# nubot-nudt/RDMNet

Hardware: AMD Instinct MI355X
Metric: scan-pairs/sec (whole node) (higher is better)
Workload: dtype f32

## Files before the change

include/rdmnet_hip.h:

```cpp
#ifndef RDMNET_HIP_H_
#define RDMNET_HIP_H_

#include <stddef.h>
#include <stdint.h>

#ifdef __cplusplus
extern "C" {
#endif

#define RDM_ABI_VERSION 2

int rdm_abi_version(void);
size_t rdm_abi_struct_size(int which);
const char* rdm_last_error(void);

int rdm_rehash_schedule(int64_t max_elems, int64_t* at_host, int64_t* buckets_host, int cap);

size_t rdm_grid_subsample_workspace_bytes(int64_t n_points, int batch);
int rdm_grid_subsample(const float* points, int64_t n_points, const int64_t* lengths, int batch,
                       float voxel_size, float* out_points, int64_t* out_lengths, void* ws,
                       size_t ws_bytes, void* stream);
int rdm_grid_subsample_form(const float* points, int64_t n_points, const int64_t* lengths, int batch, float voxel_size,
                            float* out_points, int64_t* out_lengths, void* ws, size_t ws_bytes, void* stream, int form);

// ... 51 lines not shown
size_t rdm_information_workspace_bytes(int64_t n_q, int64_t n_s);
int rdm_information_matrix(const float* q, int64_t n_q, int64_t ld_q, const float* s, int64_t n_s, int64_t ld_s,
                           const double* q_transform_host, const double* s_transform_host, double cell, double radius,
                           double* out_host, int64_t* corr_out, int64_t capacity, void* ws, size_t ws_bytes, void* stream);

size_t rdm_pose_graph_workspace_bytes(int64_t n_graphs, int64_t n_nodes, int64_t n_edges);
size_t rdm_pose_graph_workspace_bytes_pc(int64_t n_graphs, int64_t n_nodes, int64_t n_edges, int preconditioner);
int rdm_pose_graph_optimize_pc(int64_t n_graphs, const int64_t* graph_node_offsets_host, const int64_t* graph_edge_offsets_host,
                               const double* nodes, const int64_t* edges_host, const double* transforms, const double* informations,
                               const uint8_t* uncertain_host, double line_process_weight, double edge_prune_threshold,
                               int max_iterations, double gradient_tolerance, double cost_tolerance, int pcg_max_iterations,
                               double pcg_tolerance, int preconditioner, double* nodes_out, double* weights_out,
                               uint8_t* pruned_out, double* report_host, void* ws, size_t ws_bytes, void* stream);
int rdm_pose_graph_optimize(int64_t n_graphs, const int64_t* graph_node_offsets_host, const int64_t* graph_edge_offsets_host,
                            const double* nodes, const int64_t* edges_host, const double* transforms, const double* informations,
                            const uint8_t* uncertain_host, double line_process_weight, double edge_prune_threshold,
                            int max_iterations, double gradient_tolerance, double cost_tolerance, int pcg_max_iterations,
                            double pcg_tolerance, double* nodes_out, double* weights_out, uint8_t* pruned_out, double* report_host,
                            void* ws, size_t ws_bytes, void* stream);
int rdm_pose_graph_edge_terms_host(const double* source_pose, const double* target_pose, const double* transform,
                                   const double* information, double line_process_weight, int uncertain, double* out);
int rdm_pose_graph_retract_host(const double* pose, const double* delta, double* out);
int rdm_pose_graph_chain_host(int64_t n, const double* diag, const double* off, const double* rhs, double* out);
size_t rdm_pose_graph_workspace_bytes_ls(int64_t n_graphs, const int64_t* graph_node_offsets_host,
                                         const int64_t* graph_edge_offsets_host, const int64_t* edges_host, int preconditioner,
                                         int linear_solver);
int rdm_pose_graph_optimize_ls(int64_t n_graphs, const int64_t* graph_node_offsets_host, const int64_t* graph_edge_offsets_host,
                               const double* nodes, const int64_t* edges_host, const double* transforms, const double* informations,
                               const uint8_t* uncertain_host, double line_process_weight, double edge_prune_threshold,
                               int max_iterations, double gradient_tolerance, double cost_tolerance, int pcg_max_iterations,
                               double pcg_tolerance, int preconditioner, int linear_solver, double* nodes_out, double* weights_out,
                               uint8_t* pruned_out, double* report_host, void* ws, size_t ws_bytes, void* stream);
int rdm_pose_graph_direct_max_separator(void);
int64_t rdm_pose_graph_separator_host(int64_t n_nodes, int64_t n_edges, const int64_t* edges_host, int64_t* out_nodes,
                                      int64_t capacity);
int rdm_pose_graph_direct_host(int64_t n_nodes, int64_t n_edges, const int64_t* edges_host, const double* diag, const double* off,
                               const double* rhs, double* out);

size_t rdm_gemm_workspace_bytes(int64_t m, int64_t n, int batches);
int rdm_gemm(const float* a, int64_t lda, int64_t stride_a, const float* b, int64_t ldb,
             int64_t stride_b, int trans_b, float* c, int64_t ldc, int64_t stride_c, int64_t m,
             int64_t n, int64_t k, int batches, const float* bias, const float* rowdiv, int act,
             void* ws, size_t ws_bytes, void* stream);
int rdm_gemm_last_plan(int* out4_host);

int rdm_kpconv_gather(const float* q_points, int64_t m, const float* s_points, int64_t n_s,
                      const float* s_feats, int64_t c, int64_t ldf, const uint8_t* s_positive,
                      const int64_t* idx, int64_t h, int64_t ldi, const int32_t* width,
                      const float* kernel_points, float sigma, float* wf, int64_t ldw, float* nn,
                      void* stream);
int rdm_kpconv_fused_enabled(void);
int rdm_kpconv_fused_supported(int64_t c_in, int64_t c_out);
int64_t rdm_kpconv_fused_partial_rows(int64_t m, int64_t c_in);
size_t rdm_kpconv_packed_floats(int64_t c_in, int64_t c_out);
int rdm_kpconv_pack_weights(const float* w_host, int64_t c_in, int64_t c_out, float* packed_host);
int rdm_kpconv_fused(const float* q_points, int64_t m, const float* s_points, int64_t n_s, const float* s_feats,
                     int64_t c, int64_t ldf, const uint8_t* s_positive, const int64_t* idx, int64_t h, int64_t ldi,
                     const int32_t* width, const float* kernel_points, float sigma, const float* w_packed,
                     const float* bias, int64_t c_out, float* out, int64_t ldo, double* gn_partial,
                     const float* order_records, void* stream);
int rdm_kpconv_fused_form(const float* q_points, int64_t m, const float* s_points, int64_t n_s, const float* s_feats,
                          int64_t c, int64_t ldf, const uint8_t* s_positive, const int64_t* idx, int64_t h, int64_t ldi,
                          const int32_t* width, const float* kernel_points, float sigma, const float* w_packed,
                          const float* bias, int64_t c_out, float* out, int64_t ldo, double* gn_partial,
                          const float* order_records, int form, void* stream);
size_t rdm_kpconv_fused_workspace_bytes(int64_t m, int64_t c_in, int64_t c_out);
int rdm_kpconv_fused_group_norm(const float* q_points, int64_t m, const float* s_points, int64_t n_s,
                                const float* s_feats, int64_t c, int64_t ldf, const uint8_t* s_positive,
                                const int64_t* idx, int64_t h, int64_t ldi, const int32_t* width,
                                const float* kernel_points, float sigma, const float* w_packed, const float* bias,
                                int64_t c_out, int groups, const float* gamma, const float* beta, float eps, int act,
                                float* conv_out, int64_t ld_conv, float* y, int64_t ldy, void* ws, size_t ws_bytes,
                                const float* order_records, void* stream);
int rdm_kpconv_gather_ordered(const float* q_points, int64_t m, const float* s_points, int64_t n_s,
                              const float* s_feats, int64_t c, int64_t ldf, const uint8_t* s_positive,
                              const int64_t* idx, int64_t h, int64_t ldi, const int32_t* width,
                              const float* kernel_points, float sigma, float* wf, int64_t ldw, float* nn,
                              const float* order_records, void* stream);
int rdm_kpconv_gather_form(const float* q_points, int64_t m, const float* s_points, int64_t n_s,
                              const float* s_feats, int64_t c, int64_t ldf, const uint8_t* s_positive,
                              const int64_t* idx, int64_t h, int64_t ldi, const int32_t* width,
                              const float* kernel_points, float sigma, float* wf, int64_t ldw, float* nn,
                              const float* order_records, int form, void* stream);
int rdm_row_positive(const float* x, int64_t n, int64_t c, int64_t ld, uint8_t* out, void* stream);

size_t rdm_group_norm_workspace_bytes(int64_t n, int64_t c);
int rdm_group_norm(const float* x, int64_t n, int64_t c, int64_t ldx, int groups, const float* gamma,
                   const float* beta, float eps, const float* residual, int64_t ldr, int act, float* y,
                   int64_t ldy, uint8_t* positive, void* ws, size_t ws_bytes, void* stream);
int rdm_group_norm_form(const float* x, int64_t n, int64_t c, int64_t ldx, int groups, const float* gamma,
                        const float* beta, float eps, const float* residual, int64_t ldr, int act, float* y, int64_t ldy,
                        uint8_t* positive, void* ws, size_t ws_bytes, int form, void* stream);
size_t rdm_linear_group_norm_workspace_bytes(int64_t m, int64_t n);
int rdm_linear_group_norm(const float* x, int64_t ldx, const float* w, int64_t ldw, const float* bias,
                          const float* rowdiv, int64_t m, int64_t n, int64_t k, int groups, const float* gamma,
                          const float* beta, float eps, const float* residual, int64_t ldr, int act, float* lin_out,
                          int64_t ld_lin, float* y, int64_t ldy, uint8_t* positive, void* ws, size_t ws_bytes,
                          void* stream);
int rdm_patch_scores(const float* ref_feats, int64_t ld_ref, int64_t n_ref, const int64_t* ref_idx, const float* src_feats,
                     int64_t ld_src, int64_t n_src, const int64_t* src_idx, int64_t batch, int64_t side, int64_t d,
                     const float* rowdiv, float* scores, void* stream);
size_t rdm_decoder_stage_workspace_bytes(int64_t m, int64_t n, int64_t k);
int rdm_decoder_stage(const float* coarse, int64_t n_coarse, int64_t c1, int64_t ld1, const int64_t* idx, int64_t ldi,
                      const float* skip, int64_t c2, int64_t ld2, int64_t m, const float* w, int64_t ldw, const float* bias,
                      int64_t n, int groups, const float* gamma, const float* beta, float eps, int act, float* lin_out,
                      int64_t ld_lin, float* y, int64_t ldy, void* ws, size_t ws_bytes, void* stream);
int rdm_layer_norm(const float* x, int64_t n, int64_t c, int64_t ldx, const float* residual,
                   int64_t ldr, const float* gamma, const float* beta, float eps, int act, float* y,
                   int64_t ldy, void* stream);
int rdm_linear_layer_norm(const float* x, int64_t ldx, const float* w, int64_t ldw, const float* bias, int64_t m, int64_t n,
                          int64_t k, const float* residual, int64_t ldr, const float* gamma, const float* beta, float eps,
                          int act, float* y, int64_t ldy, void* stream);
int rdm_attention_tail(const float* hidden, int64_t ld_hidden, const float* x, int64_t ldx, int64_t m, int64_t d,
                       const float* wo, int64_t ld_wo, const float* bo, const float* gamma1, const float* beta1,
                       const float* w1, int64_t ld_w1, const float* b1, const float* w2, int64_t ld_w2, const float* b2,
                       const float* gamma2, const float* beta2, float eps, float* out, int64_t ld_out, void* stream);
size_t rdm_attention_tail_packed_floats(void);
int rdm_attention_tail_pack_weights(const float* wo, int64_t ld_wo, const float* w1, int64_t ld_w1, const float* w2, int64_t ld_w2,
                                    float* packed, void* stream);
int rdm_attention_tail_packed(const float* hidden, int64_t ld_hidden, const float* x, int64_t ldx, int64_t m, int64_t d,
                              const float* packed, const float* bo, const float* gamma1, const float* beta1, const float* b1,
                              const float* b2, const float* gamma2, const float* beta2, float eps, float* out, int64_t ld_out,
                              void* stream);
int rdm_gather_max(const float* x, int64_t n_s, int64_t c, int64_t ldx, const int64_t* idx, int64_t m,
                   int64_t h, int64_t ldi, const int32_t* width, float* y, int64_t ldy, void* stream);
int rdm_gather_rows(const void* x, int64_t n_src, int64_t words, int64_t ldx, const int64_t* idx, int64_t m,
                    void* y, int64_t ldy, void* stream);
int rdm_upsample_concat(const float* coarse, int64_t n_coarse, int64_t c1, int64_t ld1,
                        const int64_t* idx, int64_t ldi, const float* skip, int64_t c2, int64_t ld2,
                        int64_t m, float* y, int64_t ldy, void* stream);

int rdm_rope(float* q, int64_t ldq, float* k, int64_t ldk, const float* emb, int64_t lde, int64_t n,
             int64_t d_model, void* stream);
int rdm_attention(const float* q, int64_t ldq, const float* k, int64_t ldk, const float* v, int64_t ldv,
                  float* out, int64_t ldo, int64_t n_q, int64_t n_k, int heads, int head_dim, void* stream);
int rdm_attention_bf16(const float* q, int64_t ldq, const float* k, int64_t ldk, const float* v, int64_t ldv,
                  float* out, int64_t ldo, int64_t n_q, int64_t n_k, int heads, int head_dim, void* stream);
int rdm_attention_self_pair(const float* q, int64_t ldq, const float* k, int64_t ldk, const float* v, int64_t ldv,
                            float* out, int64_t ldo, int64_t n0, int64_t n1, int heads, int head_dim, int bf16,
                            void* stream);
int rdm_attention_topk(const float* q, int64_t ldq, const float* k, int64_t ldk, const float* v, int64_t ldv, float* out,
                       int64_t ldo, int64_t n_q, int64_t n_k, int64_t keep, int heads, int head_dim, void* stream);
int rdm_attention_self_pair_topk(const float* q, int64_t ldq, const float* k, int64_t ldk, const float* v, int64_t ldv,
                                 float* out, int64_t ldo, int64_t n0, int64_t n1, int64_t keep0, int64_t keep1, int heads,
                                 int head_dim, void* stream);
int64_t rdm_topk_count(int64_t n, double frac);

int rdm_vote_shift(const float* xyz, const float* offsets, int64_t ldo, int64_t n, float lx, float ly,
                   float lz, float* out, void* stream);
int rdm_sigmoid_column(const float* x, int64_t ldx, int64_t n, float* out, void* stream);
int rdm_l2_normalize(const float* x, int64_t ldx, int64_t n, int64_t c, float* y, int64_t ldy, void* stream);

int rdm_nms(const int64_t* idx, int64_t n, int64_t h, int64_t ldi, const int32_t* width, uint8_t* keep,
            void* stream);
int rdm_compact_indices(const uint8_t* keep, int64_t begin, int64_t end, int32_t* order, int32_t* count,
                        void* stream);

size_t rdm_point_to_node_workspace_bytes(int64_t n_points, int64_t n_nodes);
int rdm_point_to_node(const float* points, int64_t n_points, const float* nodes, int64_t n_nodes, int k,
                      int64_t* knn_idx, uint8_t* knn_mask, uint8_t* node_mask, int32_t* status, void* ws,
                      size_t ws_bytes, void* stream);
int rdm_point_to_node_pair(const float* points_a, int64_t n_a, const float* nodes_a, int64_t m_a, const float* points_b,
                           int64_t n_b, const float* nodes_b, int64_t m_b, int k, int64_t* knn_idx_a, uint8_t* knn_mask_a,
                           uint8_t* node_mask_a, int64_t* knn_idx_b, uint8_t* knn_mask_b, uint8_t* node_mask_b,
                           int32_t* status, void* ws, size_t ws_bytes, void* stream);

// ... 76 lines not shown
  int sinkhorn_iterations;
  float acceptance_radius;
  int correspondence_threshold;
  int num_refinement_steps;
  int use_vote;
  int attention_bf16;
  size_t arena_bytes;
} rdm_engine_config;

typedef struct rdm_engine_result {
  float transform[16];
  int32_t n_correspondences, n_hypotheses, best_hypothesis;
  int64_t n_ref_nodes, n_src_nodes, n_node_correspondences;
  int64_t level_sizes[5];
  int64_t level_ref_sizes[5];
  const float* ref_corr_points;
  const float* src_corr_points;
  const float* corr_scores;
  const float* transform_dev;
  size_t arena_used;
  const float* host_ref_corr_points;
  const float* host_src_corr_points;
  const float* host_corr_scores;
  int32_t n_host_correspondences;
} rdm_engine_result;

typedef struct rdm_tensor_view {
  void* data;
  int64_t rows, cols, ld;
  int dtype;
} rdm_tensor_view;

typedef struct rdm_kpconv_profile {
  int64_t m, h, c_in, c_out, pooled_channels;
  float gather_ms;
  float total_ms;
  int32_t fused;
  int32_t reserved;
} rdm_kpconv_profile;

int rdm_engine_create(const rdm_engine_config* cfg, rdm_engine** out);
void rdm_engine_destroy(rdm_engine* e);
int rdm_engine_set_param(rdm_engine* e, const char* name, const float* data_host, const int64_t* shape_host, int ndim);
int rdm_engine_finalize(rdm_engine* e);
int rdm_engine_share_params(rdm_engine* e, const rdm_engine* src);
int rdm_engine_run(rdm_engine* e, const float* ref_points, int64_t n_ref, const float* src_points, int64_t n_src,
                   rdm_engine_result* result_host, void* stream);

typedef struct rdm_data_dict {
  const float* features;  int64_t features_ld;
  const float* points[5];
  const int64_t* lengths[5];
  int64_t n_points[5], n_ref[5];
  const int64_t* neighbors[5];   int64_t neighbors_width[5],   neighbors_ld[5];   const int32_t* neighbors_count[5];
  const int64_t* subsampling[4]; int64_t subsampling_width[4], subsampling_ld[4]; const int32_t* subsampling_count[4];
  const int64_t* upsampling[4];  int64_t upsampling_width[4],  upsampling_ld[4];  const int32_t* upsampling_count[4];
  const int32_t* collate_status; int64_t n_collate_status;
} rdm_data_dict;

int rdm_engine_collate(rdm_engine* e, const float* ref_points, int64_t n_ref, const float* src_points, int64_t n_src,
                       rdm_engine_result* result_host, void* stream);

int rdm_engine_forward(rdm_engine* e, const rdm_data_dict* data, rdm_engine_result* result_host, void* stream);

int rdm_engine_collate_batch(rdm_engine* e, int n_pairs, const float* const* ref_points, const int64_t* n_ref,
                             const float* const* src_points, const int64_t* n_src, void* stream);
int rdm_engine_forward_batched(rdm_engine* e, int k, rdm_engine_result* result_host, void* stream);

int rdm_engine_run_lockstep(rdm_engine* const* engines, int n_pairs, const float* const* ref_points, const int64_t* n_ref,
                            const float* const* src_points, const int64_t* n_src, rdm_engine_result* const* results,
                            int collate_batched, void* stream);
int rdm_engine_forward_lockstep(rdm_engine* const* engines, int n_pairs, const rdm_data_dict* const* data,
                                rdm_engine_result* const* results, void* stream);
int rdm_engine_collate_lockstep(rdm_engine* const* engines, int n_pairs, const float* const* ref_points, const int64_t* n_ref,
                                const float* const* src_points, const int64_t* n_src, rdm_engine_result* const* results, void* stream);
void rdm_lockstep_stats(long long* out, int reset);
int rdm_lockstep_selftest(int n_ctx, const int* script, int len, int* log, int cap, int* rcs);
int rdm_lockstep_selftest_gpu(int n_ctx, const int* script, int len, int threads, int32_t* out, int64_t cap_slots, void* stream);
void rdm_lockstep_stats_dump(void);
int rdm_engine_reserve(rdm_engine* e, size_t bytes);
int rdm_engine_set_wait(rdm_engine* e, int sleep_us);
int rdm_engine_set_pairs_in_flight(rdm_engine* e, int n);
int rdm_engine_set_overlap(rdm_engine* e, int mode);
int rdm_engine_set_attention_topk(rdm_engine* e, int n_layers, const double* fracs);
int rdm_engine_set_fine_matching(rdm_engine* e, const rdm_fine_matching_options* options);
int rdm_engine_enable_profile(rdm_engine* e, int enable);
int rdm_engine_get_profile(rdm_engine* e, rdm_kpconv_profile* out, int cap);
int rdm_engine_keep_taps(rdm_engine* e, int enable);
int rdm_engine_get_tensor(rdm_engine* e, const char* name, rdm_tensor_view* out);
int rdm_engine_export(rdm_engine* e, int n, const char* const* names, void* const* dst, void* stream);
int rdm_engine_describe(rdm_engine* e, int n, const char* const* names, rdm_tensor_view* out);
int rdm_engine_gt_node_correspondences(rdm_engine* e, const float* transform, double pos_radius, int64_t* out_indices,
                                       float* out_overlaps, int64_t capacity, int64_t* count_host, void* stream);
int rdm_engine_feature_correspondences(rdm_engine* e, int level, int mode, int64_t* ref_idx, int64_t* src_idx, float* ref_points,
                                       float* src_points, float* dists, int64_t capacity, int64_t* count_host, void* stream);
int rdm_engine_gt_point_correspondences_count(rdm_engine* e, int level, const double* transform_host, double radius,
                                              int64_t* totals_host, void* stream);
int rdm_engine_gt_point_correspondences_fill(rdm_engine* e, int64_t* out, int64_t capacity, void* stream);
int rdm_engine_alignment_quality(rdm_engine* e, int level, const double* transform_host, double radius, double* out_host,
                                 void* stream);
int rdm_engine_information_matrix(rdm_engine* e, int level, const double* transform_host, double radius, double* out_host,
                                  int64_t* corr_out, int64_t capacity, void* stream);
int rdm_copy_device(void* dst, const void* src, size_t bytes, void* stream);

#define RDM_EVAL_RECORD_WIDTH 20
enum { RDM_EVAL_LGR = 0, RDM_EVAL_SVD = 1, RDM_EVAL_RANSAC = 2 };
typedef struct rdm_eval_options {
  int32_t method;
  int32_t num_corr;
  double acceptance_radius;
  float ransac_distance_threshold;
  int32_t ransac_n;
  int32_t ransac_iterations;
  int32_t reserved;
  uint64_t ransac_seed;
} rdm_eval_options;
size_t rdm_eval_pairs_workspace_bytes(int64_t num_pairs, int64_t total_corr, int64_t max_corr, const rdm_eval_options* options);
int rdm_eval_pairs(int64_t num_pairs, const int64_t* corr_offsets, const int64_t* corr_offsets_host, const float* ref_corr,
                   const float* src_corr, const float* corr_scores, const float* gt_transform, float* est_transform,
                   const int64_t* node_offsets, const int64_t* ref_node_corr, const int64_t* src_node_corr,
                   const int64_t* gt_offsets, const int64_t* gt_node_corr, const int64_t* node_dims,
                   const rdm_eval_options* options, double* records, void* ws, size_t ws_bytes, void* stream);

#define RDM_ROBUST_MAX_CORR 16384
#define RDM_ROBUST_STATS 6
enum { RDM_ROBUST_CLIQUE = 0, RDM_ROBUST_KCORE = 1, RDM_ROBUST_NONE = 2 };
int64_t rdm_robust_default_clique_nodes(void);
size_t rdm_robust_registration_workspace_bytes(int64_t n_corr, int inlier_selection);
int rdm_robust_registration(const float* src_corr, const float* ref_corr, int64_t n_corr, double noise_bound, double cbar2,
                            double gnc_factor, int max_iterations, double cost_threshold, int inlier_selection,
                            int64_t max_clique_nodes, double* transform, int32_t* stats, int32_t* selected, double* weights,
                            int64_t weights_capacity, int32_t* degree, int32_t* core, void* ws, size_t ws_bytes, void* stream);

#define RDM_SCAN_CONTEXT_MAX_DIM 64
#define RDM_SCAN_CONTEXT_LD 64
size_t rdm_scan_context_workspace_bytes(int64_t n_scans, int n_rings, int n_sectors);
int rdm_scan_context(const float* points, int64_t ld, int64_t n_points, const int64_t* offsets, int64_t n_scans, int n_rings,
                     int n_sectors, double max_range, double lidar_height, float* desc, float* desc_norm, uint64_t* valid, void* ws,
                     size_t ws_bytes, void* stream);
size_t rdm_scan_context_distance_workspace_bytes(int64_t n_q, int64_t n_c, int n_rings, int n_sectors);
int rdm_scan_context_distance(const float* q_desc, int64_t n_q, const float* c_desc, int64_t n_c, int n_rings, int n_sectors,
                              int64_t q_base, int64_t c_base, int64_t exclude_recent, float* best_distance, int32_t* best_index,
                              int32_t* best_shift, float* dist, int32_t* shift, void* ws, size_t ws_bytes, void* stream);

#define RDM_VOXEL_MAP_FRAC_BITS 20
#define RDM_VOXEL_MAP_MAX_CHANNELS 8
#define RDM_VOXEL_MAP_STATS 6
size_t rdm_voxel_map_bytes(int64_t capacity, int channels);
int rdm_voxel_map_reset(void* map, size_t map_bytes, int64_t capacity, int channels, void* stream);
int rdm_voxel_map_integrate(void* map, size_t map_bytes, int64_t capacity, int channels, double voxel, const float* points, int64_t ld,
                            int64_t total, const int64_t* offsets, const double* poses, int64_t n_scans, double min_range,
                            double max_range, void* stream);
int rdm_voxel_map_rehash(const void* old_map, size_t old_bytes, int64_t old_capacity, void* new_map, size_t new_bytes,
                         int64_t new_capacity, int channels, void* stream);
int rdm_voxel_map_stats(const void* map, size_t map_bytes, int64_t capacity, int channels, uint64_t* stats, void* stream);
size_t rdm_voxel_map_extract_workspace_bytes(int64_t capacity);
int rdm_voxel_map_extract(const void* map, size_t map_bytes, int64_t capacity, int channels, double voxel, int64_t min_points,
                          float* points, int32_t* counts, int32_t* cells, int64_t max_rows, int64_t* n_rows, void* ws, size_t ws_bytes,
                          void* stream);

#define RDM_VOXEL_MOMENTS_PLANES 9
#define RDM_VOXEL_MOMENTS_SHIFT 8
size_t rdm_voxel_moments_bytes(int64_t capacity);
int rdm_voxel_moments_reset(void* moments, size_t moments_bytes, int64_t capacity, void* stream);
int rdm_voxel_map_integrate_moments(void* map, size_t map_bytes, int64_t capacity, int channels, double voxel, const float* points,
                                    int64_t ld, int64_t total, const int64_t* offsets, const double* poses, int64_t n_scans,
// ... 38 lines not shown
```

rdmnet_amd/_lib.py:

```python
import ctypes
import os

_HERE = os.path.dirname(os.path.abspath(__file__))
LIB_PATH = os.environ.get('RDM_LIB_PATH') or os.path.join(_HERE, 'librdmnet_hip.so')

c_void = ctypes.c_void_p
c_i64 = ctypes.c_int64
c_int = ctypes.c_int
c_f32 = ctypes.c_float
c_size = ctypes.c_size_t

ABI_VERSION = 2


class FineMatchingOptions(ctypes.Structure):
    _fields_ = [('topk', ctypes.c_int32), ('mutual', ctypes.c_int32), ('use_dustbin', ctypes.c_int32),
                ('use_global_score', ctypes.c_int32), ('confidence_threshold', ctypes.c_float),
                ('correspondence_limit', ctypes.c_int32)]

    @classmethod
    def of(cls, topk=1, mutual=False, use_dustbin=True, confidence_threshold=0.0, use_global_score=False,
           correspondence_limit=None):
        return cls(int(topk), int(bool(mutual)), int(bool(use_dustbin)), int(bool(use_global_score)), float(confidence_threshold),
                   0 if correspondence_limit is None else int(correspondence_limit))


class EvalOptions(ctypes.Structure):
    METHODS = {'lgr': 0, 'svd': 1, 'ransac': 2}
    _fields_ = [('method', ctypes.c_int32), ('num_corr', ctypes.c_int32), ('acceptance_radius', ctypes.c_double),
                ('ransac_distance_threshold', ctypes.c_float), ('ransac_n', ctypes.c_int32),
                ('ransac_iterations', ctypes.c_int32), ('reserved', ctypes.c_int32), ('ransac_seed', ctypes.c_uint64)]

    @classmethod
    def of(cls, method='lgr', num_corr=None, acceptance_radius=0.6, distance_threshold=0.3, ransac_n=4, num_iterations=50000,
           seed=0):
        if method not in cls.METHODS:
            raise ValueError(f'Unsupported registration method: {method}.')
        return cls(cls.METHODS[method], 0 if num_corr is None else int(num_corr), float(acceptance_radius),
                   float(distance_threshold), int(ransac_n), int(num_iterations), 0, int(seed))


ROBUST_SELECTIONS = {'clique': 0, 'kcore': 1, 'none': 2}
ROBUST_MAX_CORR = 16384
ROBUST_STATS = ('num_selected', 'valid', 'exact', 'iterations', 'translation_inliers', 'edges')

SCAN_CONTEXT_MAX_DIM = 64
SCAN_CONTEXT_LD = 64

VOXEL_MAP_FRAC_BITS = 20
VOXEL_MAP_MAX_CHANNELS = 8
VOXEL_MAP_STATS = ('occupied', 'integrated', 'skipped_nonfinite', 'skipped_range', 'out_of_extent', 'dropped_full')
VOXEL_MOMENTS_PLANES = 9
VOXEL_OBSERVATIONS_MAX_SCANS = 64

EVAL_RECORD_WIDTH = 20
EVAL_FIELDS = ('num_corr', 'residual', 'inlier_ratio', 'inlier_ratio_0.3', 'inlier_ratio_0.1', 'overlap', 'precision', 'rre', 'rte',
               'rx', 'ry', 'rz', 'inliers', 'inliers_0.3', 'inliers_0.1', 'overlap_rows', 'hit_cells', 'pred_cells', 'gt_cells',
               'bad_indices')

SIGNATURES = {
    'rdm_abi_version': (c_int, []),
    'rdm_abi_struct_size': (c_size, [c_int]),
    'rdm_last_error': (ctypes.c_char_p, []),
    'rdm_rehash_schedule': (c_int, [c_i64, c_void, c_void, c_int]),
    'rdm_grid_subsample_workspace_bytes': (c_size, [c_i64, c_int]),
    'rdm_grid_subsample': (c_int, [c_void, c_i64, c_void, c_int, c_f32, c_void, c_void, c_void, c_size,
                                   c_void]),
    'rdm_grid_subsample_form': (c_int, [c_void, c_i64, c_void, c_int, c_f32, c_void, c_void, c_void, c_size,
                                        c_void, c_int]),
    'rdm_radius_neighbors_workspace_bytes': (c_size, [c_i64, c_i64, c_int]),
    'rdm_radius_neighbors': (c_int, [c_void, c_i64, c_void, c_i64, c_void, c_void, c_int, c_f32, c_int,
                                     c_void, c_void, c_void, c_void, c_void, c_size, c_void]),
    'rdm_radius_grid_workspace_bytes': (c_size, [c_i64]),
    'rdm_radius_grid_build': (c_int, [c_void, c_i64, c_void, c_int, c_f32, c_void, c_size, c_void]),
    'rdm_radius_grid_query': (c_int, [c_void, c_size, c_i64, c_void, c_i64, c_void, c_int, c_f32, c_int, c_void, c_void,
                                      c_void, c_void, c_void, c_size, c_void]),
    'rdm_gemm_workspace_bytes': (c_size, [c_i64, c_i64, c_int]),
    'rdm_gemm': (c_int, [c_void, c_i64, c_i64, c_void, c_i64, c_i64, c_int, c_void, c_i64, c_i64, c_i64, c_i64,
                         c_i64, c_int, c_void, c_void, c_int, c_void, c_size, c_void]),
    'rdm_gemm_last_plan': (c_int, [c_void]),
    'rdm_kpconv_gather': (c_int, [c_void, c_i64, c_void, c_i64, c_void, c_i64, c_i64, c_void, c_void, c_i64,
                                  c_i64, c_void, c_void, c_f32, c_void, c_i64, c_void, c_void]),
    'rdm_kpconv_gather_ordered': (c_int, [c_void, c_i64, c_void, c_i64, c_void, c_i64, c_i64, c_void, c_void, c_i64,
                                          c_i64, c_void, c_void, c_f32, c_void, c_i64, c_void, c_void, c_void]),
    'rdm_kpconv_gather_form': (c_int, [c_void, c_i64, c_void, c_i64, c_void, c_i64, c_i64, c_void, c_void, c_i64,
                                       c_i64, c_void, c_void, c_f32, c_void, c_i64, c_void, c_void, c_int, c_void]),
    'rdm_kpconv_fused_enabled': (c_int, []),
    'rdm_kpconv_fused_supported': (c_int, [c_i64, c_i64]),
    'rdm_kpconv_fused_partial_rows': (c_i64, [c_i64, c_i64]),
    'rdm_kpconv_packed_floats': (c_size, [c_i64, c_i64]),
    'rdm_kpconv_pack_weights': (c_int, [c_void, c_i64, c_i64, c_void]),
    'rdm_kpconv_fused': (c_int, [c_void, c_i64, c_void, c_i64, c_void, c_i64, c_i64, c_void, c_void, c_i64, c_i64, c_void, c_void,
                                 c_f32, c_void, c_void, c_i64, c_void, c_i64, c_void, c_void, c_void]),
    'rdm_kpconv_fused_form': (c_int, [c_void, c_i64, c_void, c_i64, c_void, c_i64, c_i64, c_void, c_void, c_i64, c_i64, c_void, c_void,
                                      c_f32, c_void, c_void, c_i64, c_void, c_i64, c_void, c_void, c_int, c_void]),
    'rdm_kpconv_fused_workspace_bytes': (c_size, [c_i64, c_i64, c_i64]),
    'rdm_kpconv_fused_group_norm': (c_int, [c_void, c_i64, c_void, c_i64, c_void, c_i64, c_i64, c_void, c_void, c_i64, c_i64, c_void,
                                            c_void, c_f32, c_void, c_void, c_i64, c_int, c_void, c_void, c_f32, c_int, c_void, c_i64,
                                            c_void, c_i64, c_void, c_size, c_void, c_void]),
    'rdm_voxel_downsample_workspace_bytes': (c_size, [c_i64]),
    'rdm_voxel_downsample': (c_int, [c_void, c_i64, c_i64, c_int, ctypes.c_double, c_void, c_i64, c_void, c_void, c_void,
                                     c_size, c_void]),
    'rdm_ransac_workspace_bytes': (c_size, [c_int]),
    'rdm_ransac_correspondences': (c_int, [c_void, c_void, c_i64, c_f32, c_int, c_int, ctypes.c_uint64, c_void, c_void, c_void,
                                           c_void, c_void, c_size, c_void]),
    'rdm_icp_workspace_bytes': (c_size, [c_i64, c_i64]),
    'rdm_icp_point_to_point': (c_int, [c_void, c_i64, c_i64, c_void, c_i64, c_i64, ctypes.c_double, c_void, c_int, ctypes.c_double,
                                       ctypes.c_double, c_void, c_void, c_void, c_void, c_void, c_size, c_void]),
    'rdm_icp_correspondences': (c_int, [c_void, c_i64, c_void, c_i64, c_i64, ctypes.c_double, c_void, c_void, c_void, c_size,
                                        c_void]),
    'rdm_ball_workspace_bytes': (c_size, [c_i64, c_i64]),
    'rdm_ball_count': (c_int, [c_void, c_i64, c_i64, c_void, c_i64, c_i64, c_void, ctypes.c_double, c_void, c_void, c_void, c_void,
                               c_void, c_size, c_void]),
    'rdm_ball_fill': (c_int, [c_void, c_i64, c_i64, c_i64, c_void, c_i64, c_void, c_size, c_void]),
    'rdm_nearest_workspace_bytes': (c_size, [c_i64, c_i64]),
    'rdm_nearest': (c_int, [c_void, c_i64, c_i64, c_void, c_i64, c_i64, c_void, c_void, ctypes.c_double, ctypes.c_double, c_void,
                            c_void, c_void, c_void, c_size, c_void]),
    'rdm_realign_error': (c_int, [c_void, c_i64, c_i64, c_void, c_void, c_void, c_void, c_size, c_void]),
    'rdm_information_workspace_bytes': (c_size, [c_i64, c_i64]),
    'rdm_information_matrix': (c_int, [c_void, c_i64, c_i64, c_void, c_i64, c_i64, c_void, c_void, ctypes.c_double, ctypes.c_double,
                                       c_void, c_void, c_i64, c_void, c_size, c_void]),
    'rdm_pose_graph_workspace_bytes': (c_size, [c_i64, c_i64, c_i64]),
    'rdm_pose_graph_optimize': (c_int, [c_i64, c_void, c_void, c_void, c_void, c_void, c_void, c_void, ctypes.c_double, ctypes.c_double,
                                        c_int, ctypes.c_double, ctypes.c_double, c_int, ctypes.c_double, c_void, c_void, c_void, c_void,
                                        c_void, c_size, c_void]),
    'rdm_pose_graph_workspace_bytes_pc': (c_size, [c_i64, c_i64, c_i64, c_int]),
    'rdm_pose_graph_optimize_pc': (c_int, [c_i64, c_void, c_void, c_void, c_void, c_void, c_void, c_void, ctypes.c_double,
                                           ctypes.c_double, c_int, ctypes.c_double, ctypes.c_double, c_int, ctypes.c_double, c_int,
                                           c_void, c_void, c_void, c_void, c_void, c_size, c_void]),
    'rdm_pose_graph_chain_host': (c_int, [c_i64, c_void, c_void, c_void, c_void]),
    'rdm_pose_graph_workspace_bytes_ls': (c_size, [c_i64, c_void, c_void, c_void, c_int, c_int]),
    'rdm_pose_graph_optimize_ls': (c_int, [c_i64, c_void, c_void, c_void, c_void, c_void, c_void, c_void, ctypes.c_double,
                                           ctypes.c_double, c_int, ctypes.c_double, ctypes.c_double, c_int, ctypes.c_double, c_int, c_int,
                                           c_void, c_void, c_void, c_void, c_void, c_size, c_void]),
    'rdm_pose_graph_direct_max_separator': (c_int, []),
    'rdm_pose_graph_separator_host': (c_i64, [c_i64, c_i64, c_void, c_void, c_i64]),
    'rdm_pose_graph_direct_host': (c_int, [c_i64, c_i64, c_void, c_void, c_void, c_void, c_void]),
    'rdm_pose_graph_edge_terms_host': (c_int, [c_void, c_void, c_void, c_void, ctypes.c_double, c_int, c_void]),
    'rdm_pose_graph_retract_host': (c_int, [c_void, c_void, c_void]),
    'rdm_neighbor_histogram': (c_int, [c_void, c_i64, c_void, c_int, c_void]),
    'rdm_radius_grid_records': (c_void, [c_void, c_size, c_i64]),
    'rdm_row_positive': (c_int, [c_void, c_i64, c_i64, c_i64, c_void, c_void]),
    'rdm_group_norm_workspace_bytes': (c_size, [c_i64, c_i64]),
    'rdm_group_norm': (c_int, [c_void, c_i64, c_i64, c_i64, c_int, c_void, c_void, c_f32, c_void, c_i64, c_int,
                               c_void, c_i64, c_void, c_void, c_size, c_void]),
    'rdm_group_norm_form': (c_int, [c_void, c_i64, c_i64, c_i64, c_int, c_void, c_void, c_f32, c_void, c_i64, c_int,
                                    c_void, c_i64, c_void, c_void, c_size, c_int, c_void]),
    'rdm_linear_group_norm_workspace_bytes': (c_size, [c_i64, c_i64]),
    'rdm_linear_group_norm': (c_int, [c_void, c_i64, c_void, c_i64, c_void, c_void, c_i64, c_i64, c_i64, c_int, c_void, c_void,
                                      c_f32, c_void, c_i64, c_int, c_void, c_i64, c_void, c_i64, c_void, c_void, c_size, c_void]),
    'rdm_patch_scores': (c_int, [c_void, c_i64, c_i64, c_void, c_void, c_i64, c_i64, c_void, c_i64, c_i64, c_i64, c_void, c_void,
                                 c_void]),
    'rdm_decoder_stage_workspace_bytes': (c_size, [c_i64, c_i64, c_i64]),
    'rdm_decoder_stage': (c_int, [c_void, c_i64, c_i64, c_i64, c_void, c_i64, c_void, c_i64, c_i64, c_i64, c_void, c_i64, c_void,
                                  c_i64, c_int, c_void, c_void, c_f32, c_int, c_void, c_i64, c_void, c_i64, c_void, c_size, c_void]),
    'rdm_layer_norm': (c_int, [c_void, c_i64, c_i64, c_i64, c_void, c_i64, c_void, c_void, c_f32, c_int, c_void,
                               c_i64, c_void]),
    'rdm_linear_layer_norm': (c_int, [c_void, c_i64, c_void, c_i64, c_void, c_i64, c_i64, c_i64, c_void, c_i64, c_void, c_void,
                                      c_f32, c_int, c_void, c_i64, c_void]),
    'rdm_attention_tail': (c_int, [c_void, c_i64, c_void, c_i64, c_i64, c_i64, c_void, c_i64, c_void, c_void, c_void, c_void, c_i64,
                                   c_void, c_void, c_i64, c_void, c_void, c_void, c_f32, c_void, c_i64, c_void]),
    'rdm_attention_tail_packed_floats': (c_size, []),
    'rdm_attention_tail_pack_weights': (c_int, [c_void, c_i64, c_void, c_i64, c_void, c_i64, c_void, c_void]),
    'rdm_attention_tail_packed': (c_int, [c_void, c_i64, c_void, c_i64, c_i64, c_i64, c_void, c_void, c_void, c_void, c_void, c_void,
                                          c_void, c_void, c_f32, c_void, c_i64, c_void]),
    'rdm_gather_max': (c_int, [c_void, c_i64, c_i64, c_i64, c_void, c_i64, c_i64, c_i64, c_void, c_void, c_i64,
                               c_void]),
    'rdm_upsample_concat': (c_int, [c_void, c_i64, c_i64, c_i64, c_void, c_i64, c_void, c_i64, c_i64, c_i64,
                                    c_void, c_i64, c_void]),
    'rdm_gather_rows': (c_int, [c_void, c_i64, c_i64, c_i64, c_void, c_i64, c_void, c_i64, c_void]),
    'rdm_rope': (c_int, [c_void, c_i64, c_void, c_i64, c_void, c_i64, c_i64, c_i64, c_void]),
    'rdm_attention': (c_int, [c_void, c_i64, c_void, c_i64, c_void, c_i64, c_void, c_i64, c_i64, c_i64, c_int, c_int,
                              c_void]),
    'rdm_attention_bf16': (c_int, [c_void, c_i64, c_void, c_i64, c_void, c_i64, c_void, c_i64, c_i64, c_i64, c_int, c_int,
                              c_void]),
    'rdm_attention_self_pair': (c_int, [c_void, c_i64, c_void, c_i64, c_void, c_i64, c_void, c_i64, c_i64, c_i64, c_int, c_int,
                                        c_int, c_void]),
    'rdm_attention_topk': (c_int, [c_void, c_i64, c_void, c_i64, c_void, c_i64, c_void, c_i64, c_i64, c_i64, c_i64, c_int, c_int,
                                   c_void]),
    'rdm_attention_self_pair_topk': (c_int, [c_void, c_i64, c_void, c_i64, c_void, c_i64, c_void, c_i64, c_i64, c_i64, c_i64, c_i64,
                                             c_int, c_int, c_void]),
    'rdm_topk_count': (c_i64, [c_i64, ctypes.c_double]),
    'rdm_vote_shift': (c_int, [c_void, c_void, c_i64, c_i64, c_f32, c_f32, c_f32, c_void, c_void]),
    'rdm_sigmoid_column': (c_int, [c_void, c_i64, c_i64, c_void, c_void]),
    'rdm_l2_normalize': (c_int, [c_void, c_i64, c_i64, c_i64, c_void, c_i64, c_void]),
    'rdm_nms': (c_int, [c_void, c_i64, c_i64, c_i64, c_void, c_void, c_void]),
    'rdm_compact_indices': (c_int, [c_void, c_i64, c_i64, c_void, c_void, c_void]),
    'rdm_point_to_node_workspace_bytes': (c_size, [c_i64, c_i64]),
    'rdm_point_to_node': (c_int, [c_void, c_i64, c_void, c_i64, c_int, c_void, c_void, c_void, c_void, c_void,
                                  c_size, c_void]),
    'rdm_point_to_node_pair': (c_int, [c_void, c_i64, c_void, c_i64, c_void, c_i64, c_void, c_i64, c_int, c_void, c_void, c_void,
                                       c_void, c_void, c_void, c_void, c_void, c_size, c_void]),
    'rdm_coarse_matching_workspace_bytes': (c_size, [c_i64, c_i64]),
    'rdm_coarse_matching': (c_int, [c_void, c_i64, c_i64, c_i64, c_void, c_void, c_int, c_int, c_void, c_void, c_void,
                                    c_void, c_void, c_size, c_void]),
    'rdm_coarse_matching_features_workspace_bytes': (c_size, [c_i64, c_i64]),
    'rdm_coarse_matching_features': (c_int, [c_void, c_i64, c_i64, c_void, c_i64, c_i64, c_i64, c_void, c_void, c_int, c_int,
                                             c_void, c_void, c_void, c_void, c_void, c_size, c_void]),
    'rdm_gt_node_correspondences_workspace_bytes': (c_size, [c_i64, c_i64]),
    'rdm_gt_node_correspondences': (c_int, [c_void, c_i64, c_void, c_i64, c_void, c_void, c_i64, c_void, c_void, c_i64, c_int,
                                            c_void, c_void, c_void, c_void, c_void, ctypes.c_double, c_void, c_void, c_i64,
                                            c_void, c_void, c_void, c_size, c_void]),
    'rdm_sinkhorn': (c_int, [c_void, c_i64, c_i64, c_i64, c_void, c_void, c_void, c_int, c_void, c_void]),
    'rdm_lgr_workspace_bytes': (c_size, [c_i64]),
    'rdm_lgr': (c_int, [c_void, c_void, c_void, c_void, c_void, c_i64, c_i64, c_f32, c_int, c_int, c_void, c_void,
                        c_void, c_void, c_void, c_void, c_size, c_void]),
    'rdm_lgr_options_capacity': (c_i64, [c_i64, c_i64, c_void]),
    'rdm_lgr_options_workspace_bytes': (c_size, [c_i64, c_i64, c_void]),
    'rdm_lgr_options': (c_int, [c_void, c_i64, c_void, c_void, c_void, c_void, c_void, c_i64, c_i64, c_f32, c_int, c_int, c_void,
                                c_void, c_void, c_void, c_void, c_void, c_void, c_size, c_void]),
    'rdm_engine_create': (c_int, [c_void, c_void]),
    'rdm_engine_destroy': (None, [c_void]),
    'rdm_engine_set_param': (c_int, [c_void, ctypes.c_char_p, c_void, c_void, c_int]),
    'rdm_engine_finalize': (c_int, [c_void]),
    'rdm_engine_share_params': (c_int, [c_void, c_void]),
    'rdm_engine_run': (c_int, [c_void, c_void, c_i64, c_void, c_i64, c_void, c_void]),
    'rdm_engine_collate': (c_int, [c_void, c_void, c_i64, c_void, c_i64, c_void, c_void]),
    'rdm_engine_forward': (c_int, [c_void, c_void, c_void, c_void]),
    'rdm_engine_collate_batch': (c_int, [c_void, c_int, c_void, c_void, c_void, c_void, c_void]),
    'rdm_engine_forward_batched': (c_int, [c_void, c_int, c_void, c_void]),
    'rdm_engine_run_lockstep': (c_int, [c_void, c_int, c_void, c_void, c_void, c_void, c_void, c_int, c_void]),
    'rdm_engine_forward_lockstep': (c_int, [c_void, c_int, c_void, c_void, c_void]),
    'rdm_engine_collate_lockstep': (c_int, [c_void, c_int, c_void, c_void, c_void, c_void, c_void, c_void]),
    'rdm_lockstep_stats': (None, [c_void, c_int]),
    'rdm_lockstep_stats_dump': (None, []),
    'rdm_lockstep_selftest': (c_int, [c_int, c_void, c_int, c_void, c_int, c_void]),
    'rdm_lockstep_selftest_gpu': (c_int, [c_int, c_void, c_int, c_int, c_void, c_i64, c_void]),
    'rdm_engine_reserve': (c_int, [c_void, c_size]),
    'rdm_engine_set_wait': (c_int, [c_void, c_int]),
    'rdm_engine_set_pairs_in_flight': (c_int, [c_void, c_int]),
    'rdm_engine_set_overlap': (c_int, [c_void, c_int]),
    'rdm_engine_set_attention_topk': (c_int, [c_void, c_int, c_void]),
    'rdm_engine_set_fine_matching': (c_int, [c_void, c_void]),
    'rdm_engine_enable_profile': (c_int, [c_void, c_int]),
    'rdm_engine_get_profile': (c_int, [c_void, c_void, c_int]),
    'rdm_engine_keep_taps': (c_int, [c_void, c_int]),
    'rdm_engine_get_tensor': (c_int, [c_void, ctypes.c_char_p, c_void]),
    'rdm_engine_describe': (c_int, [c_void, c_int, c_void, c_void]),
    'rdm_engine_export': (c_int, [c_void, c_int, c_void, c_void, c_void]),
    'rdm_engine_gt_node_correspondences': (c_int, [c_void, c_void, ctypes.c_double, c_void, c_void, c_i64, c_void, c_void]),
    'rdm_feature_match_workspace_bytes': (c_size, [c_i64, c_i64, c_int]),
    'rdm_feature_match': (c_int, [c_void, c_i64, c_i64, c_void, c_i64, c_i64, c_i64, c_int, c_void, c_void, c_void, c_void, c_void,
                                  c_void, c_size, c_void]),
    'rdm_feature_match_select': (c_int, [c_int, c_void, c_void, c_void, c_void, c_i64, c_i64, c_void, c_void, c_void, c_void, c_void]),
    'rdm_engine_feature_correspondences': (c_int, [c_void, c_int, c_int, c_void, c_void, c_void, c_void, c_void, c_i64, c_void,
                                                   c_void]),
    'rdm_engine_gt_point_correspondences_count': (c_int, [c_void, c_int, c_void, ctypes.c_double, c_void, c_void]),
    'rdm_engine_gt_point_correspondences_fill': (c_int, [c_void, c_void, c_i64, c_void]),
    'rdm_engine_alignment_quality': (c_int, [c_void, c_int, c_void, ctypes.c_double, c_void, c_void]),
    'rdm_engine_information_matrix': (c_int, [c_void, c_int, c_void, ctypes.c_double, c_void, c_void, c_i64, c_void]),
    'rdm_copy_device': (c_int, [c_void, c_void, c_size, c_void]),
    'rdm_eval_pairs_workspace_bytes': (c_size, [c_i64, c_i64, c_i64, c_void]),
    'rdm_eval_pairs': (c_int, [c_i64, c_void, c_void, c_void, c_void, c_void, c_void, c_void, c_void, c_void, c_void, c_void,
                               c_void, c_void, c_void, c_void, c_void, c_size, c_void]),
    'rdm_robust_default_clique_nodes': (c_i64, []),
    'rdm_robust_registration_workspace_bytes': (c_size, [c_i64, c_int]),
    'rdm_robust_registration': (c_int, [c_void, c_void, c_i64, ctypes.c_double, ctypes.c_double, ctypes.c_double, c_int,
                                        ctypes.c_double, c_int, c_i64, c_void, c_void, c_void, c_void, c_i64, c_void, c_void,
                                        c_void, c_size, c_void]),
    'rdm_scan_context_workspace_bytes': (c_size, [c_i64, c_int, c_int]),
    'rdm_scan_context': (c_int, [c_void, c_i64, c_i64, c_void, c_i64, c_int, c_int, ctypes.c_double, ctypes.c_double, c_void, c_void,
                                 c_void, c_void, c_size, c_void]),
    'rdm_scan_context_distance_workspace_bytes': (c_size, [c_i64, c_i64, c_int, c_int]),
    'rdm_scan_context_distance': (c_int, [c_void, c_i64, c_void, c_i64, c_int, c_int, c_i64, c_i64, c_i64, c_void, c_void, c_void,
                                          c_void, c_void, c_void, c_size, c_void]),
    'rdm_voxel_map_bytes': (c_size, [c_i64, c_int]),
    'rdm_voxel_map_reset': (c_int, [c_void, c_size, c_i64, c_int, c_void]),
    'rdm_voxel_map_integrate': (c_int, [c_void, c_size, c_i64, c_int, ctypes.c_double, c_void, c_i64, c_i64, c_void, c_void, c_i64,
                                        ctypes.c_double, ctypes.c_double, c_void]),
    'rdm_voxel_map_rehash': (c_int, [c_void, c_size, c_i64, c_void, c_size, c_i64, c_int, c_void]),
    'rdm_voxel_map_stats': (c_int, [c_void, c_size, c_i64, c_int, c_void, c_void]),
    'rdm_voxel_map_extract_workspace_bytes': (c_size, [c_i64]),
    'rdm_voxel_map_extract': (c_int, [c_void, c_size, c_i64, c_int, ctypes.c_double, c_i64, c_void, c_void, c_void, c_i64, c_void,
                                      c_void, c_size, c_void]),
    'rdm_voxel_moments_bytes': (c_size, [c_i64]),
    'rdm_voxel_moments_reset': (c_int, [c_void, c_size, c_i64, c_void]),
    'rdm_voxel_map_integrate_moments': (c_int, [c_void, c_size, c_i64, c_int, ctypes.c_double, c_void, c_i64, c_i64, c_void, c_void,
                                                c_i64, ctypes.c_double, ctypes.c_double, c_void, c_size, c_void]),
    'rdm_voxel_moments_rehash': (c_int, [c_void, c_size, c_i64, c_void, c_size, c_void, c_size, c_i64, c_void, c_size, c_int, c_void]),
    'rdm_voxel_map_extract_moments': (c_int, [c_void, c_size, c_i64, c_int, c_void, c_size, ctypes.c_double, c_i64, c_void, c_void,
                                              c_void, c_void, c_i64, c_void, c_void, c_size, c_void]),
    'rdm_voxel_map_register_workspace_bytes': (c_size, [c_i64]),
    'rdm_voxel_map_register': (c_int, [c_void, c_size, c_i64, c_int, c_void, c_size, ctypes.c_double, c_void, c_i64, c_i64, c_void, c_void,
                                       c_i64, ctypes.c_double, ctypes.c_double, ctypes.c_double, c_i64, c_int, c_int, ctypes.c_double,
                                       ctypes.c_double, c_void, c_void, c_void, c_void, c_void, c_void, c_size, c_void]),
    'rdm_voxel_observations_bytes': (c_size, [c_i64]),
    'rdm_voxel_observations_reset': (c_int, [c_void, c_size, c_i64, c_void]),
    'rdm_voxel_map_integrate_observed': (c_int, [c_void, c_size, c_i64, c_int, ctypes.c_double, c_void, c_i64, c_i64, c_void, c_void,
                                                 c_i64, ctypes.c_double, ctypes.c_double, c_void, c_size, c_void, c_size, c_i64, c_void]),
    'rdm_voxel_observations_rehash': (c_int, [c_void, c_size, c_i64, c_void, c_size, c_void, c_size, c_i64, c_void, c_size, c_int, c_void]),
    'rdm_voxel_map_extract_observations': (c_int, [c_void, c_size, c_i64, c_int, c_void, c_size, ctypes.c_double, c_i64, c_void, c_void,
                                                   c_void, c_i64, c_void, c_void, c_size, c_void]),
    'rdm_voxel_map_prune': (c_int, [c_void, c_size, c_i64, c_void, c_size, c_void, c_size, c_i64, c_int, c_i64, c_i64, c_void]),
}



_lib = None


def build():
    import subprocess
    subprocess.run(['make', '-C', os.path.join(_HERE, 'csrc'), '-j8'], check=True)


def lib():
    global _lib
    if _lib is None:
        if not os.path.exists(LIB_PATH):
            raise RuntimeError(
                f'{LIB_PATH} is missing: build it with `make -C rdmnet_amd/csrc` '
                '(or __graft_entry__.build()); there is no CPU fallback')
        handle = ctypes.CDLL(LIB_PATH)
        for name, (res, args) in SIGNATURES.items():
# ... 34 lines not shown
```

rdmnet_amd/csrc/engine.hip:

```cpp
#include <algorithm>
#include <cmath>
#include <cstring>
#include <atomic>
#include <chrono>
#include <functional>
#include <map>
#include <memory>
#include <string>
#include <vector>

#include "../../include/rdmnet_hip.h"
#include <ctime>

#include "common.h"
#include "internal.h"
#include "lockstep.h"

namespace {

using namespace rdm;

struct Mat {
  float* p = nullptr;
  int64_t rows = 0, cols = 0, ld = 0;
// ... 1 lines not shown
  Mat rows_from(int64_t r0, int64_t n) const { return Mat{p + r0 * ld, n, cols, ld}; }
};

struct HostParam {
  std::vector<int64_t> shape;
  std::vector<float> data;
};

struct Linear {
  float* b = nullptr;
  float* wt = nullptr;
  float* bias = nullptr;
  float* packed = nullptr;
  int64_t in = 0, out = 0, kpad = 0, ldb = 0;
};

inline int64_t pad4(int64_t n) { return (n + 3) / 4 * 4; }

struct ParamSet {
  std::map<std::string, Linear> lin;
  std::map<std::string, float*> vec;
  std::vector<void*> owned;
  int device = -1;
  ParamSet() = default;
  ParamSet(const ParamSet&) = delete;
  ParamSet& operator=(const ParamSet&) = delete;
  ~ParamSet() {
    for (void* p : owned) (void)hipFree(p);
  }
};

struct Level {
  float* pts = nullptr;
  int64_t n = 0;
  int64_t* lengths = nullptr;
  int64_t n_ref = 0;
};
struct Table {
  int64_t* idx = nullptr;
  bool i32 = false;
  int64_t rows = 0, width = 0;
  int64_t ld = 0;
  int32_t* flags = nullptr;
  int64_t stride() const { return ld ? ld : width; }
};

struct Grid {
  void* ws = nullptr;
  size_t bytes = 0;
  int64_t n_s = 0;
};
struct PairPyramid {
  Level lv[5];
  Table nb[5], sub[4], up[4];
  Grid grids[5];
  int32_t* flags = nullptr;
  int calls = 0;
};

}

struct rdm_engine {
  rdm_engine_config cfg;
  int device = -1;
  std::map<std::string, HostParam> host;
  std::shared_ptr<ParamSet> params = std::make_shared<ParamSet>();
  char* arena = nullptr;
  size_t arena_cap = 0, arena_off = 0;
  bool arena_exhausted = false, arena_fixed = false;
  void* pinned = nullptr;
  void* pinned_dev = nullptr;
  int64_t host_corr_cap = 0;
  int wait_sleep_us = 0;
  bool finalized = false;
  std::map<std::string, rdm_tensor_view> taps;
  bool keep_taps = false;
  bool collate_only = false;
  std::vector<double> topk_fracs;
  bool has_fm = false;
  rdm_fine_matching_options fm{1, 0, 1, 0, 0.f, 0};
  int pairs_in_flight = 1;
  int overlap_mode = 1;
  hipStream_t side = nullptr;
  std::map<hipStream_t, bool> side_ok;
  std::vector<PairPyramid> batch;
  std::vector<int64_t> batch_n_ref, batch_n_src;
  size_t arena_base = 0;
  bool profile = false;
  bool profile_shapes_only = false;
  std::vector<hipEvent_t> events;
  std::vector<rdm_kpconv_profile> prof;
  int prof_layers = 0;
  struct GtInputs {
    bool valid = false;
    const float* nodes[2] = {nullptr, nullptr};
    int64_t m[2] = {0, 0};
    const float* pf[2] = {nullptr, nullptr};
    int64_t nf[2] = {0, 0};
    const int64_t* knn[2] = {nullptr, nullptr};
    const uint8_t* km[2] = {nullptr, nullptr};
    const uint8_t* nm[2] = {nullptr, nullptr};
    int k = 0;
    const float* ff = nullptr; int64_t ff_ld = 0;
    const float* fc = nullptr; int64_t fc_ld = 0;
    int d = 0;
    const float* p0[2] = {nullptr, nullptr};
    int64_t n0[2] = {0, 0};
    struct Ball {
      bool pending = false;
      const float* ref = nullptr;
      int64_t n = 0, m = 0, count = 0;
      char* ws = nullptr;
      size_t ws_bytes = 0, off_before = 0;
    } ball;
    float est[16] = {1, 0, 0, 0, 0, 1, 0, 0, 0, 0, 1, 0, 0, 0, 0, 1};
  } gt;

  template <typename T>
  T* alloc(size_t count) {
    size_t bytes = align_up(count * sizeof(T) + 16);
    if (arena_off + bytes > arena_cap) return nullptr;
    T* r = reinterpret_cast<T*>(arena + arena_off);
    arena_off += bytes;
    return r;
  }
  Mat mat(int64_t rows, int64_t cols) {
    Mat m;
    m.rows = rows; m.cols = cols; m.ld = pad4(cols);
    m.p = alloc<float>(static_cast<size_t>(rows > 0 ? rows : 1) * m.ld);
    return m;
  }
};

namespace {

#define ENG_CHECK(...)             \
  do {                             \
    int _rc = (__VA_ARGS__);       \
    if (_rc != 0) return _rc;      \
  } while (0)
#define ENG_ALLOC(ptr)                                             \
  do {                                                             \
    if ((ptr) == nullptr) {                                        \
      set_error("rdm_engine: activation arena exhausted (%zu B)", e->arena_cap); \
      e->arena_exhausted = true;                                   \
      return RDM_ERR_WORKSPACE;                                    \
    }                                                              \
  } while (0)

struct Run {
  rdm_engine* e;
  hipStream_t st;
  void* ws;
  size_t ws_bytes;
  int groups;
};

void tap(Run& r, const char* name, const void* p, int64_t rows, int64_t cols, int64_t ld, int dtype) {
  if (!r.e->keep_taps) return;
  rdm_tensor_view v;
  v.data = const_cast<void*>(p); v.rows = rows; v.cols = cols; v.ld = ld; v.dtype = dtype;
  r.e->taps[name] = v;
}
void tap(Run& r, const char* name, const Mat& m) { tap(r, name, m.p, m.rows, m.cols, m.ld, 0); }

const Linear* lin_param(Run& r, const std::string& name) {
// ... 98 lines not shown
  if (need > ws_bytes) {
    ws = e->alloc<char>(need);
    ENG_ALLOC(ws);
    ws_bytes = need;
  }
  return rdm::decoder_stage_cols(coarse.p, coarse.rows, coarse.cols, coarse.ld, up_idx, up_ld, skip.p, skip.cols, skip.ld, m, L.b,
                                 L.ldb, L.bias, L.out, n, r.groups, g, b, 1e-5f, 2, t.p, t.ld, norm_name ? y.p : nullptr,
                                 norm_name ? y.ld : 0, ws, ws_bytes, r.st);
}

int layer_norm(Run& r, const std::string& name, const Mat& x, const Mat* res, int act, Mat& y, bool alloc_out = true) {
  lockstep_align();
  rdm_engine* e = r.e;
  if (alloc_out) {
    y = e->mat(x.rows, x.cols);
    ENG_ALLOC(y.p);
  }
  return rdm_layer_norm(x.p, x.rows, x.cols, x.ld, res ? res->p : nullptr, res ? res->ld : 0, vecp(r, name + ".weight"),
                        vecp(r, name + ".bias"), 1e-5f, act, y.p, y.ld, r.st);
}

int layer_event(rdm_engine* e, int k, hipStream_t st) {
  if (e->profile_shapes_only) return RDM_OK;
  if (lockstep_active()) {
    lockstep_event(e->events[k], st);
    return RDM_OK;
  }
  RDM_HIP_CHECK(hipEventRecord(e->events[k], st));
  return RDM_OK;
}

int kpconv(Run& r, const std::string& name, const Mat& x, const uint8_t* x_pos, const Level& q, const Level& s,
           const Table& t, float sigma, const std::string& norm_name, Mat& y, const float* order,
           const Mat* pool_src = nullptr, Mat* pool_out = nullptr) {
  lockstep_align();
  rdm_engine* e = r.e;
  const Linear* Wp = lin_param(r, name + ".weights");
  if (!Wp) return RDM_ERR_ARG;
  const Linear& W = *Wp;
  const int64_t cin = x.cols, kdim = cin == 1 ? 16 : 15 * cin;
  const int i32 = t.i32 ? 1 : 0;
  const int li = e->prof_layers;
  const bool prof = e->profile && (e->profile_shapes_only ? li < 16 : 3 * li + 2 < static_cast<int>(e->events.size()));
  auto end_profile = [&](int fused) -> int {
    ENG_CHECK(layer_event(e, 3 * li + 2, r.st));
    rdm_kpconv_profile p;
    p.m = q.n; p.h = t.width; p.c_in = cin; p.c_out = W.out; p.pooled_channels = pool_src ? pool_src->cols : 0;
    p.gather_ms = p.total_ms = 0.f;
    p.fused = fused; p.reserved = 0;
    e->prof.push_back(p);
    e->prof_layers++;
    return RDM_OK;
  };
  if (W.packed && rdm_kpconv_fused_enabled()) {
    float *gam, *bet;
    ENG_CHECK(norm_params(r, norm_name + ".norm", &gam, &bet));
    Mat conv = e->mat(q.n, W.out);
    y = e->mat(q.n, W.out);
    ENG_ALLOC(conv.p); ENG_ALLOC(y.p);
    RDM_REQUIRE(rdm_kpconv_fused_workspace_bytes(q.n, cin, W.out) <= r.ws_bytes, "rdm_engine: scratch too small");
    if (prof) ENG_CHECK(layer_event(e, 3 * li, r.st));
    const int nblk = static_cast<int>(rdm_kpconv_fused_partial_rows(q.n, cin));
    double* gn_partial = static_cast<double*>(r.ws);
    const size_t stat_bytes = align_up(static_cast<size_t>(nblk) * 2 * W.out * sizeof(double));
    ENG_CHECK(kpconv_fused_impl(q.pts, q.n, s.pts, s.n, x.p, cin, x.ld, x_pos, t.idx, t.width, t.stride(), t.flags,
                                vecp(r, name + ".kernel_points"), sigma, W.packed, W.bias, W.out, conv.p, conv.ld, gn_partial, order, 0,
                                i32, r.st));
    if (prof) ENG_CHECK(layer_event(e, 3 * li + 1, r.st));
    ENG_CHECK(group_norm_finish(gn_partial, nblk, conv.p, q.n, W.out, conv.ld, r.groups, gam, bet, 1e-5f, nullptr, 0, 2, y.p, y.ld,
                                nullptr, static_cast<char*>(r.ws) + stat_bytes, r.ws_bytes - stat_bytes, r.st));
    if (pool_src) {
      *pool_out = e->mat(q.n, pool_src->cols);
      ENG_ALLOC(pool_out->p);
      ENG_CHECK(gather_max_ordered(pool_src->p, pool_src->rows, pool_src->cols, pool_src->ld, t.idx, q.n, t.width, t.stride(),
                                   t.flags, pool_out->p, pool_out->ld, order, i32, r.st));
    }
    if (prof) ENG_CHECK(end_profile(1));
    return RDM_OK;
  }
  Mat wf = e->mat(q.n, kdim);
  ENG_ALLOC(wf.p);
  float* nn = e->alloc<float>(q.n > 0 ? q.n : 1);
  ENG_ALLOC(nn);
  if (prof) ENG_CHECK(layer_event(e, 3 * li, r.st));
  ENG_CHECK(kpconv_gather_impl(q.pts, q.n, s.pts, s.n, x.p, cin, x.ld, x_pos, t.idx, t.width, t.stride(), t.flags,
                               vecp(r, name + ".kernel_points"), sigma, wf.p, wf.ld, nn, order, i32, r.st));
  if (prof) ENG_CHECK(layer_event(e, 3 * li + 1, r.st));
  Mat conv = e->mat(q.n, W.out);
  ENG_ALLOC(conv.p);
  const size_t gemm_ws = rdm_gemm_workspace_bytes(q.n, W.out, 1);
  const size_t stat_bytes = align_up(static_cast<size_t>(gemm_stats_max_blocks(q.n)) * 2 * W.out * sizeof(double));
  RDM_REQUIRE(gemm_ws + stat_bytes + rdm_group_norm_workspace_bytes(q.n, W.out) <= r.ws_bytes, "rdm_engine: scratch too small");
  double* gn_partial = reinterpret_cast<double*>(static_cast<char*>(r.ws) + gemm_ws);
  int gn_blocks = 0;
  ENG_CHECK(gemm_with_stats(wf.p, wf.ld, W.b, W.ldb, conv.p, conv.ld, q.n, W.out, W.kpad, W.bias, nn, r.ws, gemm_ws,
                            gn_partial, &gn_blocks, r.st));
  if (pool_src) {
    *pool_out = e->mat(q.n, pool_src->cols);
    ENG_ALLOC(pool_out->p);
    ENG_CHECK(gather_max_ordered(pool_src->p, pool_src->rows, pool_src->cols, pool_src->ld, t.idx, q.n, t.width, t.stride(),
                                   t.flags, pool_out->p, pool_out->ld, order, i32, r.st));
  }
  if (prof) ENG_CHECK(end_profile(0));
  y = e->mat(q.n, W.out);
  ENG_ALLOC(y.p);
  float *gam, *bet;
  ENG_CHECK(norm_params(r, norm_name + ".norm", &gam, &bet));
  return group_norm_finish(gn_partial, gn_blocks, conv.p, q.n, W.out, conv.ld, r.groups, gam, bet, 1e-5f, nullptr, 0, 2, y.p,
                           y.ld, nullptr, static_cast<char*>(r.ws) + gemm_ws + stat_bytes, r.ws_bytes - gemm_ws - stat_bytes,
                           r.st);
}

int linear_ln(Run& r, const std::string& lin, const std::string& norm, const Mat& x, const Mat& res, Mat& y, bool alloc_out) {
  lockstep_align();
  rdm_engine* e = r.e;
  const Linear* Lp = lin_param(r, lin);
  if (!Lp) return RDM_ERR_ARG;
  const Linear& L = *Lp;
  if (L.wt && L.out == 128) {
    if (alloc_out) {
      y = e->mat(x.rows, L.out);
      ENG_ALLOC(y.p);
    }
    return rdm_linear_layer_norm(x.p, x.ld, L.wt, L.kpad, L.bias, x.rows, L.out, L.kpad, res.p, res.ld, vecp(r, norm + ".weight"),
                                 vecp(r, norm + ".bias"), 1e-5f, 0, y.p, y.ld, r.st);
  }
  Mat h;
  ENG_CHECK(linear(r, lin, x, h));
  return layer_norm(r, norm, h, &res, 0, y, alloc_out);
}

int attention_tail(Run& r, const std::string& p, const Mat& hid, const Mat& x, Mat out) {
  lockstep_align();
  rdm_engine* e = r.e;
  auto lo = e->params->lin.find(p + ".attention.linear"), l1 = e->params->lin.find(p + ".output.expand"), l2 = e->params->lin.find(p + ".output.squeeze");
  if (lo != e->params->lin.end() && l1 != e->params->lin.end() && l2 != e->params->lin.end() && lo->second.wt && l1->second.wt && l2->second.wt &&
      lo->second.out == 128 && lo->second.kpad == 128 && l1->second.out == 256 && l1->second.kpad == 128 &&
      l2->second.out == 128 && l2->second.kpad == 256) {
    const Linear &Lo = lo->second, &L1 = l1->second, &L2 = l2->second;
    auto pk = e->params->vec.find(p + ".__tail_packed");
    static const bool unpacked = ::rdm::dev_knob("RDM_TAIL_UNPACKED") != nullptr;
    if (pk != e->params->vec.end() && !unpacked)
      return rdm_attention_tail_packed(hid.p, hid.ld, x.p, x.ld, hid.rows, 128, pk->second, Lo.bias, vecp(r, p + ".attention.norm.weight"),
                                       vecp(r, p + ".attention.norm.bias"), L1.bias, L2.bias, vecp(r, p + ".output.norm.weight"),
                                       vecp(r, p + ".output.norm.bias"), 1e-5f, out.p, out.ld, r.st);
    return rdm_attention_tail(hid.p, hid.ld, x.p, x.ld, hid.rows, 128, Lo.wt, Lo.kpad, Lo.bias, vecp(r, p + ".attention.norm.weight"),
                              vecp(r, p + ".attention.norm.bias"), L1.wt, L1.kpad, L1.bias, L2.wt, L2.kpad, L2.bias,
                              vecp(r, p + ".output.norm.weight"), vecp(r, p + ".output.norm.bias"), 1e-5f, out.p, out.ld, r.st);
  }
  Mat y, z1;
  ENG_CHECK(linear_ln(r, p + ".attention.linear", p + ".attention.norm", hid, x, y, true));
  ENG_CHECK(linear(r, p + ".output.expand", y, z1, 1));
  return linear_ln(r, p + ".output.squeeze", p + ".output.norm", z1, y, out, false);
}

int thdroformer(Run& r, const std::string& name, const Mat& pts4, const Mat& x, int64_t n0, int num_layers, Mat out,
                const std::function<int()>* after_two = nullptr, const std::vector<double>* topk = nullptr) {
  rdm_engine* e = r.e;
  const int heads = e->cfg.num_heads;
  const int64_t N = x.rows, n1 = N - n0;
  Mat emb, f;
  ENG_CHECK(linear(r, name + ".embedding.proj", pts4, emb));
  ENG_CHECK(linear(r, name + ".in_proj", x, f));
  const int64_t d = f.cols;
  const int hd = static_cast<int>(d / heads);
  const auto attend = e->cfg.attention_bf16 ? rdm_attention_bf16 : rdm_attention;
  for (int i = 0; i < 2 * num_layers; ++i) {
    const std::string p = name + ".transformer.layers." + std::to_string(i);
    Mat fnew = e->mat(N, d), hid = e->mat(N, d);
    ENG_ALLOC(fnew.p); ENG_ALLOC(hid.p);
    if (i % 2 == 0) {
      Mat qkv;
      ENG_CHECK(linear(r, p + ".qkv", f, qkv));
      Mat q = qkv.cols_from(0, d), k = qkv.cols_from(d, d), v = qkv.cols_from(2 * d, d);
      ENG_CHECK(rdm_rope(q.p, q.ld, k.p, k.ld, emb.p, emb.ld, N, d, r.st));
      const size_t self_idx = static_cast<size_t>(i / 2);
      if (topk && self_idx < topk->size() && (*topk)[self_idx] >= 0) {
        const double f = (*topk)[self_idx];
        ENG_CHECK(rdm_attention_self_pair_topk(q.p, q.ld, k.p, k.ld, v.p, v.ld, hid.p, hid.ld, n0, n1, rdm_topk_count(n0, f),
// ... 400 lines not shown
  RDM_REQUIRE(e && bytes >= (size_t(1) << 20), "rdm_engine_reserve: at least 1 MiB");
  RDM_HIP_CHECK(hipDeviceSynchronize());
  e->batch.clear();
  e->arena_base = 0;
  e->gt.valid = false;
  RDM_HIP_CHECK(hipFree(e->arena));
  e->arena = nullptr;
  e->arena_cap = bytes;
  e->arena_fixed = false;
  const hipError_t err = hipMalloc(reinterpret_cast<void**>(&e->arena), e->arena_cap);
  if (err != hipSuccess) {
    e->arena_cap = 0;
    set_error("rdm_engine_reserve: hipMalloc(%zu) failed: %s", bytes, hipGetErrorString(err));
    return RDM_ERR_HIP;
  }
  return RDM_OK;
}

extern "C" int rdm_engine_set_wait(rdm_engine* e, int sleep_us) {
  RDM_REQUIRE(e && sleep_us >= 0, "rdm_engine_set_wait: bad arguments");
  e->wait_sleep_us = sleep_us;
  return RDM_OK;
}

extern "C" int rdm_engine_set_pairs_in_flight(rdm_engine* e, int n) {
  RDM_REQUIRE(e && n >= 1, "rdm_engine_set_pairs_in_flight: bad arguments");
  e->pairs_in_flight = n;
  return RDM_OK;
}

extern "C" int rdm_engine_set_fine_matching(rdm_engine* e, const rdm_fine_matching_options* o) {
  RDM_REQUIRE(e, "rdm_engine_set_fine_matching: null engine");
  if (!o) {
    e->has_fm = false;
    return RDM_OK;
  }
  const int K = std::max(e->cfg.points_in_patch, 1);
  RDM_REQUIRE(o->topk >= 1 && o->topk <= K + (o->use_dustbin ? 1 : 0), "rdm_engine_set_fine_matching: topk = %d is outside [1, %d]",
              o->topk, K + (o->use_dustbin ? 1 : 0));
  RDM_REQUIRE(o->confidence_threshold >= 0.f, "rdm_engine_set_fine_matching: confidence_threshold = %g is not >= 0",
              static_cast<double>(o->confidence_threshold));
  RDM_REQUIRE(o->correspondence_limit >= 0, "rdm_engine_set_fine_matching: correspondence_limit = %d (0 = none, or >= 1)",
              o->correspondence_limit);
  const int64_t cap = rdm_lgr_options_capacity(std::max(e->cfg.num_correspondences, 1), K, o);
  if (cap > e->host_corr_cap) {
    int device = -1;
    RDM_HIP_CHECK(hipGetDevice(&device));
    RDM_REQUIRE(device == e->device, "rdm_engine_set_fine_matching: the engine belongs to device %d, current is %d", e->device, device);
    void* pinned = nullptr;
    void* pinned_dev = nullptr;
    RDM_HIP_CHECK(hipHostMalloc(&pinned, 4096 + static_cast<size_t>(cap) * 7 * sizeof(float), hipHostMallocMapped));
    const hipError_t err = hipHostGetDevicePointer(&pinned_dev, pinned, 0);
    if (err != hipSuccess) {
      (void)hipHostFree(pinned);
      set_error("rdm_engine_set_fine_matching: hipHostGetDevicePointer failed: %s", hipGetErrorString(err));
      return RDM_ERR_HIP;
    }
    RDM_HIP_CHECK(hipDeviceSynchronize());
    if (e->pinned) (void)hipHostFree(e->pinned);
    e->pinned = pinned;
    e->pinned_dev = pinned_dev;
    e->host_corr_cap = cap;
  }
  e->fm = *o;
  e->has_fm = true;
  return RDM_OK;
}

extern "C" int rdm_engine_set_attention_topk(rdm_engine* e, int n_layers, const double* fracs) {
  RDM_REQUIRE(e && n_layers >= 0 && (n_layers == 0 || fracs), "rdm_engine_set_attention_topk: bad arguments");
  RDM_REQUIRE(n_layers == 0 || !e->cfg.attention_bf16, "rdm_engine_set_attention_topk: no top-k variant of bf16 attention");
  for (int i = 0; i < n_layers; ++i)
    RDM_REQUIRE(fracs[i] <= 1.0 && !std::isnan(fracs[i]), "rdm_engine_set_attention_topk: fraction %d is %g (not <= 1)", i, fracs[i]);
  e->topk_fracs.assign(fracs, fracs + n_layers);
  return RDM_OK;
}

extern "C" int rdm_engine_set_overlap(rdm_engine* e, int mode) {
  RDM_REQUIRE(e && mode >= 0 && mode <= 2, "rdm_engine_set_overlap: bad arguments");
  e->overlap_mode = mode;
  return RDM_OK;
}

extern "C" int rdm_engine_get_profile(rdm_engine* e, rdm_kpconv_profile* out, int cap) {
  RDM_REQUIRE(e && out && cap >= 0, "rdm_engine_get_profile: bad arguments");
  const int n = std::min<int>(cap, static_cast<int>(e->prof.size()));
  for (int i = 0; i < n; ++i) out[i] = e->prof[i];
  return static_cast<int>(e->prof.size());
}

extern "C" int rdm_engine_keep_taps(rdm_engine* e, int enable) {
  RDM_REQUIRE(e, "rdm_engine_keep_taps: null engine");
  e->keep_taps = enable != 0;
  return RDM_OK;
}

extern "C" int rdm_engine_get_tensor(rdm_engine* e, const char* name, rdm_tensor_view* out) {
  RDM_REQUIRE(e && name && out, "rdm_engine_get_tensor: null pointer");
  auto it = e->taps.find(name);
  if (it == e->taps.end()) {
    set_error("rdm_engine_get_tensor: no tensor named %s (call rdm_engine_keep_taps first)", name);
    return RDM_ERR_ARG;
  }
  *out = it->second;
  return RDM_OK;
}

namespace {

struct PadGuard {
  explicit PadGuard(unsigned b) { rdm::gemm_set_lds_pad(b); }
  ~PadGuard() { rdm::gemm_set_lds_pad(0); }
};
struct CollateOnly {
  rdm_engine* e;
  bool keep_before;
  explicit CollateOnly(rdm_engine* eng) : e(eng), keep_before(eng->keep_taps) { e->keep_taps = e->collate_only = true; }
  ~CollateOnly() { e->collate_only = false; e->keep_taps = keep_before; }
};

int gs_multi_levels() {
  static const int n = [] { const char* v = ::rdm::dev_knob("RDM_GS_MULTI_LEVELS"); return v ? atoi(v) : 1; }();
  return n;
}

struct SearchQueue {
  std::vector<char> buf = std::vector<char>(radius_redo_queue_bytes());
  int queued = 0;
  hipStream_t st;
  explicit SearchQueue(hipStream_t s) : st(s) { radius_redo_queue_reset(buf.data()); }
  int flush() {
    queued = 0;
    return radius_redo_flush(buf.data(), st);
  }
};

int search(rdm_engine* e, SearchQueue& sq, const Level& q, const Grid& g, float rad, int limit, bool i32, int32_t* status,
           Table& t) {
  if (sq.queued == 16) ENG_CHECK(sq.flush());
  t.rows = q.n; t.width = limit; t.flags = status;
  t.i32 = i32;
  t.idx = reinterpret_cast<int64_t*>(e->alloc<char>(static_cast<size_t>(q.n > 0 ? q.n : 1) * limit * (i32 ? 4 : 8)));
  ENG_ALLOC(t.idx);
  unsigned char* redo_flags = e->alloc<unsigned char>(static_cast<size_t>(q.n > 0 ? q.n : 1));
  ENG_ALLOC(redo_flags);
  ++sq.queued;
  return radius_grid_query_deferred(g.ws, g.bytes, g.n_s, q.pts, q.n, q.lengths, 2, rad, limit, t.idx, nullptr, t.flags,
                                    t.flags + 1, redo_flags, sq.buf.data(), i32 ? 1 : 0, sq.st);
}

int search_pyramid(rdm_engine* e, PairPyramid& py, bool full, bool nb0_done, SearchQueue& sq) {
  const rdm_engine_config& c = e->cfg;
  auto row = [&py] { return py.flags + 2 * py.calls++; };
  float radius = c.init_radius;
  for (int i = 0; i < 5; ++i, radius *= 2.f) {
    const Level* lv = py.lv;
    if (!(nb0_done && i == 0)) ENG_CHECK(search(e, sq, lv[i], py.grids[i], radius, c.neighbor_limits[i], !full, row(), py.nb[i]));
    if (i < 4) ENG_CHECK(search(e, sq, lv[i + 1], py.grids[i], radius, c.neighbor_limits[i], !full, row(), py.sub[i]));
    if (i > 0 && (full || i > 1))
      ENG_CHECK(search(e, sq, lv[i - 1], py.grids[i], radius, full ? c.neighbor_limits[i] : 1, false, row(), py.up[i - 1]));
  }
  return RDM_OK;
}

int build_level_grids(rdm_engine* e, PairPyramid* pys, int n, int first, int last, hipStream_t st) {
  const float* gp[8];
// ... 1305 lines not shown
```

rdmnet_amd/csrc/gemm.hip:

```cpp
#include "../../include/rdmnet_hip.h"
#include <cmath>
#include <cstdlib>

#include "common.h"
#include "internal.h"
#include "lockstep.h"

namespace {

using namespace rdm;

typedef float f32x16 __attribute__((ext_vector_type(16)));
typedef float f32x4_t __attribute__((ext_vector_type(4)));

struct GemmArgs {
  const float* A = nullptr;
  const float* B = nullptr;
  float* C = nullptr;
  const float* bias = nullptr;
  const float* rowdiv = nullptr;
  int M = 0, N = 0, K = 0;
  int lda = 0, ldb = 0, ldc = 0;
  long long sa = 0, sb = 0, sc = 0;
  int act = 0;
  int splits = 1;
  float* part = nullptr;
  double* stats = nullptr;
  const float* A2 = nullptr;
  const int64_t* aidx = nullptr;
  int lda2 = 0, ldi = 0, c1 = 0, n_coarse = 0;
  const int64_t* bidx = nullptr;
  int n_b = 0;
  const float* seed = nullptr;
  const int64_t* sidx = nullptr;
  int ld_seed = 0, ldsi = 0, n_seed = 0;
  int xcd_tiles = 0;
#ifdef RDM_GEMM_TIMING
  unsigned long long* clk = nullptr;
#endif
};
#ifdef RDM_GEMM_TIMING
#define GEMM_STAMP(k) do { if (blockIdx.x == 0 && blockIdx.y == 0 && blockIdx.z == 0 && threadIdx.x == 0) g.clk[k] = __builtin_amdgcn_s_memtime(); } while (0)
#else
#define GEMM_STAMP(k) do { } while (0)
#endif

__device__ __forceinline__ float apply_act(float v, int act) {
  if (act == 1) return v > 0.f ? v : 0.f;
  if (act == 2) return v > 0.f ? v : 0.1f * v;
  return v;
}

template <int BM, int BN, int WM, int WN, int BK, bool TRANS_B, int PF, bool CAT = false, bool SEED = false>
__device__ __forceinline__ void gemm_kernel_body(const dim3 blockIdx, const dim3 gridDim, GemmArgs g) {
  (void)blockIdx; (void)gridDim;
  constexpr int TM = BM / WM, TN = BN / WN, FM = TM / 32, FN = TN / 32;
  static_assert(WM * WN == 4 && TM % 32 == 0 && TN % 32 == 0, "bad tile");
  static_assert(!SEED || (!CAT && !TRANS_B), "seeded accumulators: plain operands only");
  constexpr int LDA_S = BM + 1, LDB_S = TRANS_B ? BN + 1 : BN + 4;
  constexpr int CR = BM < 64 ? BM : 64;
  constexpr int LDC_S = BN + 4;
  constexpr int TPR = BN / 4;
  constexpr int RPI = 256 / TPR;
  constexpr int kBytesAB = (2 * BK * LDA_S + 2 * BK * LDB_S) * 4, kBytesC = CR * LDC_S * 4, kBytesStat = RPI * BN * 2 * 8;
  constexpr int kBytes = kBytesAB > kBytesC ? (kBytesAB > kBytesStat ? kBytesAB : kBytesStat) : (kBytesC > kBytesStat ? kBytesC : kBytesStat);
  static_assert((2 * BK * LDA_S * 4) % 16 == 0 && CR % RPI == 0, "tile layout");
  __shared__ __attribute__((aligned(16))) char smem[kBytes];
  float (*As)[BK][LDA_S] = reinterpret_cast<float (*)[BK][LDA_S]>(smem);
  float (*Bs)[BK][LDB_S] = reinterpret_cast<float (*)[BK][LDB_S]>(smem + 2 * BK * LDA_S * 4);
  float (*Cs)[LDC_S] = reinterpret_cast<float (*)[LDC_S]>(smem);
  double (*stat_red)[1][2] = reinterpret_cast<double (*)[1][2]>(smem);

  const int tid = threadIdx.x, lane = tid & 63, wave = tid >> 6;
  const int wm = wave / WN, wn = wave % WN;
  int tile_x = blockIdx.x, tile_y = blockIdx.y;
  if (g.xcd_tiles) {
    const int nblk = gridDim.x * gridDim.y, lin = blockIdx.y * gridDim.x + blockIdx.x;
    const int q = nblk / 8, rr = nblk % 8, xcd = lin % 8, within = lin / 8;
    const int logical = (xcd < rr ? xcd * (q + 1) : rr * (q + 1) + (xcd - rr) * q) + within;
    tile_x = logical % gridDim.x;
    tile_y = logical / gridDim.x;
  }
  const int m0 = tile_y * BM, n0 = tile_x * BN;
  GEMM_STAMP(0);
  const int batch = blockIdx.z / g.splits, split = blockIdx.z % g.splits;
  const float* A = g.A + batch * g.sa;
  const float* B = g.B + batch * g.sb;

  const int ktiles = (g.K + BK - 1) / BK;
  const int per = (ktiles + g.splits - 1) / g.splits;
  const int kt0 = split * per, kt1 = min(ktiles, kt0 + per);

  constexpr int A_N4 = BM * BK / 4;
  constexpr int A_V = (A_N4 + 255) / 256;
  constexpr int KC4 = BK / 4;
  constexpr int B_N4 = BK * BN / 4;
  constexpr int B_V = (B_N4 + 255) / 256;
  static_assert(PF == 1 || PF == 2, "one or two register stages");
  float4 ra0[A_V], rb0[B_V], ra1[PF == 2 ? A_V : 1], rb1[PF == 2 ? B_V : 1];
  long long cat_row[CAT ? A_V : 1], cat_brow[CAT && TRANS_B ? B_V : 1];
  if constexpr (CAT && !TRANS_B) {
#pragma unroll
    for (int i = 0; i < A_V; ++i) {
      const int row = (tid + i * 256) / (BK / 4);
      const long long id = g.aidx[static_cast<long long>(min(m0 + row, g.M - 1)) * g.ldi];
      cat_row[i] = (id >= 0 && id < g.n_coarse) ? id : -1;
    }
  }
  if constexpr (CAT && TRANS_B) {
    A = g.A;
    B = g.B;
    int any_a = 0, any_b = 0;
#pragma unroll
    for (int i = 0; i < A_V; ++i) {
      const int row = (tid + i * 256) / (BK / 4);
      const long long id = (m0 + row < g.M && (A_N4 % 256 == 0 || tid + i * 256 < A_N4)) ? g.aidx[static_cast<long long>(batch) * g.M + m0 + row] : -1;
      cat_row[i] = (id >= 0 && id < g.n_coarse) ? id : -1;
      any_a |= cat_row[i] >= 0;
    }
#pragma unroll
    for (int i = 0; i < B_V; ++i) {
      const int row = (tid + i * 256) / (BK / 4);
      const long long id = (n0 + row < g.N && (B_N4 % 256 == 0 || tid + i * 256 < B_N4)) ? g.bidx[static_cast<long long>(batch) * g.N + n0 + row] : -1;
      cat_brow[i] = (id >= 0 && id < g.n_b) ? id : -1;
      any_b |= cat_brow[i] >= 0;
    }
    any_a = __syncthreads_or(any_a);
    any_b = __syncthreads_or(any_b);
    if (!any_a || !any_b) {
      float* Cz = g.C + batch * g.sc;
      for (int e = tid; e < BM * BN; e += 256) {
        const int r = m0 + e / BN, cc = n0 + e % BN;
        if (r < g.M && cc < g.N) Cz[static_cast<long long>(r) * g.ldc + cc] = 0.f;
      }
      return;
    }
  }

  auto load_tiles = [&](float4 (&ra)[A_V], float4 (&rb)[B_V], int kt, int p0 = 0, int p1 = 1 << 20) {
    const int k0 = min(kt, kt1 - 1) * BK;
#pragma unroll
    for (int i = 0; i < A_V; ++i) {
      if (i < p0 || i >= p1) continue;
      const int idx = tid + i * 256;
      const int row = idx / KC4, kc = (idx % KC4) * 4;
      if constexpr (CAT && TRANS_B) {
        ra[i] = *reinterpret_cast<const float4*>(A + max(cat_row[i], 0ll) * g.lda + min(k0 + kc, g.K - 4));
      } else if constexpr (CAT) {
        const float* src = k0 < g.c1 ? A + max(cat_row[i], 0ll) * g.lda + (k0 + kc)
                                     : g.A2 + static_cast<long long>(min(m0 + row, g.M - 1)) * g.lda2 + min(k0 - g.c1 + kc, g.K - g.c1 - 4);
        ra[i] = *reinterpret_cast<const float4*>(src);
      } else {
      ra[i] = *reinterpret_cast<const float4*>(A + static_cast<long long>(min(m0 + row, g.M - 1)) * g.lda + min(k0 + kc, g.K - 4));
      }
    }
#pragma unroll
    for (int i = 0; i < B_V; ++i) {
      if (A_V + i < p0 || A_V + i >= p1) continue;
      const int idx = tid + i * 256;
      if (TRANS_B) {
        const int row = idx / KC4, kc = (idx % KC4) * 4;
        if constexpr (CAT) {
          rb[i] = *reinterpret_cast<const float4*>(B + max(cat_brow[i], 0ll) * g.ldb + min(k0 + kc, g.K - 4));
        } else {
        rb[i] = *reinterpret_cast<const float4*>(B + static_cast<long long>(min(n0 + row, g.N - 1)) * g.ldb + min(k0 + kc, g.K - 4));
        }
      } else {
        const int k = idx / (BN / 4), n4 = (idx % (BN / 4)) * 4;
        rb[i] = *reinterpret_cast<const float4*>(B + static_cast<long long>(min(k0 + k, g.K - 1)) * g.ldb + min(n0 + n4, g.ldb - 4));
      }
    }
  };
  auto masked = [](const float4& v, bool ok) { return make_float4(ok ? v.x : 0.f, ok ? v.y : 0.f, ok ? v.z : 0.f, ok ? v.w : 0.f); };
  auto store_tiles = [&](const float4 (&ra)[A_V], const float4 (&rb)[B_V], int buf, int kt, int p0 = 0, int p1 = 1 << 20) {
    const int k0 = min(kt, kt1 - 1) * BK;
#pragma unroll
    for (int i = 0; i < A_V; ++i) {
      if (i < p0 || i >= p1) continue;
      const int idx = tid + i * 256;
      const int row = idx / KC4, kc = (idx % KC4) * 4;
      if (A_N4 % 256 != 0 && idx >= A_N4) continue;
      bool a_ok = m0 + row < g.M && k0 + kc < g.K;
      if constexpr (CAT && TRANS_B) a_ok = a_ok && cat_row[i] >= 0;
      else if constexpr (CAT) a_ok = a_ok && (k0 >= g.c1 || cat_row[i] >= 0);
      const float4 v = masked(ra[i], a_ok);
      As[buf][kc + 0][row] = v.x;
      As[buf][kc + 1][row] = v.y;
      As[buf][kc + 2][row] = v.z;
      As[buf][kc + 3][row] = v.w;
    }
    if (TRANS_B) {
#pragma unroll
      for (int i = 0; i < B_V; ++i) {
        if (A_V + i < p0 || A_V + i >= p1) continue;
        const int idx = tid + i * 256;
        const int row = idx / KC4, kc = (idx % KC4) * 4;
        if (B_N4 % 256 != 0 && idx >= B_N4) continue;
        bool b_ok = n0 + row < g.N && k0 + kc < g.K;
        if constexpr (CAT) b_ok = b_ok && cat_brow[i] >= 0;
        const float4 v = masked(rb[i], b_ok);
        Bs[buf][kc + 0][row] = v.x;
        Bs[buf][kc + 1][row] = v.y;
        Bs[buf][kc + 2][row] = v.z;
        Bs[buf][kc + 3][row] = v.w;
      }
    } else {
#pragma unroll
      for (int i = 0; i < B_V; ++i) {
        if (A_V + i < p0 || A_V + i >= p1) continue;
        const int idx = tid + i * 256;
        const int k = idx / (BN / 4), n4 = (idx % (BN / 4)) * 4;
        if (B_N4 % 256 != 0 && idx >= B_N4) continue;
        *reinterpret_cast<float4*>(&Bs[buf][k][n4]) = masked(rb[i], k0 + k < g.K && n0 + n4 < g.ldb);
      }
    }
  };

  const bool partial = g.splits > 1;
  const int c4 = (tid % TPR) * 4, rsub = tid / TPR;
  const int gcol = n0 + c4;
  float bv[4] = {0.f, 0.f, 0.f, 0.f};
  float rdv[BM / RPI];
  if (!partial && g.bias)
#pragma unroll
    for (int e = 0; e < 4; ++e) bv[e] = gcol + e < g.N ? g.bias[gcol + e] : 0.f;
#pragma unroll
  for (int q = 0; q < BM / RPI; ++q) rdv[q] = (!partial && g.rowdiv) ? g.rowdiv[min(m0 + q * RPI + rsub, g.M - 1)] : 1.f;

  const int lk = lane >> 5, li = lane & 31;
  f32x16 acc[FM][FN];
#pragma unroll
  for (int i = 0; i < FM; ++i)
#pragma unroll
    for (int j = 0; j < FN; ++j)
#pragma unroll
      for (int r = 0; r < 16; ++r) acc[i][j][r] = 0.f;
  long long seed_row[SEED ? FM : 1][SEED ? 16 : 1];
  if constexpr (SEED) {
#pragma unroll
    for (int i = 0; i < FM; ++i)
#pragma unroll
      for (int r = 0; r < 16; ++r) {
        const int row = m0 + wm * TM + i * 32 + (r & 3) + 8 * (r >> 2) + 4 * lk;
        const long long id = g.sidx[static_cast<long long>(min(row, g.M - 1)) * g.ldsi];
        seed_row[i][r] = (row < g.M && id >= 0 && id < g.n_seed) ? id : -1;
      }
  }
  constexpr int HK = BK / 2, HS = HK / 2;
  float af_lo[HS][FM], bf_lo[HS][FN], af_hi[HS][FM], bf_hi[HS][FN];
  auto read_kstep = [&](float (&af)[HS][FM], float (&bf)[HS][FN], int buf, int kbase, int s) {
#pragma unroll
    for (int i = 0; i < FM; ++i) af[s][i] = As[buf][kbase + 2 * s + lk][wm * TM + i * 32 + li];
#pragma unroll
    for (int j = 0; j < FN; ++j) bf[s][j] = Bs[buf][kbase + 2 * s + lk][wn * TN + j * 32 + li];
  };
  auto read_half = [&](float (&af)[HS][FM], float (&bf)[HS][FN], int buf, int kbase) {
#pragma unroll
    for (int s = 0; s < HS; ++s) read_kstep(af, bf, buf, kbase, s);
  };
  constexpr int NCH = HS * FM * FN, NP = A_V + B_V;
  auto step = [&](auto& fa, auto& fb, const auto& na, const auto& nb, int kt, int buf) {
#pragma unroll
    for (int c = 0; c < NCH; ++c) {
      const int s = c / (FM * FN), i = (c / FN) % FM, j = c % FN;
      acc[i][j] = __builtin_amdgcn_mfma_f32_32x32x2f32(af_lo[s][i], bf_lo[s][j], acc[i][j], 0, 0, 0);
      if (c % (FM * FN) == 0) read_kstep(af_hi, bf_hi, buf, HK, s);
      load_tiles(fa, fb, kt + PF, NCH >= NP ? (c < NP ? c : NP) : (c * NP) / NCH, NCH >= NP ? (c < NP ? c + 1 : NP) : ((c + 1) * NP) / NCH);
      store_tiles(na, nb, buf ^ 1, kt + 1, NCH >= NP ? (c >= NCH - NP ? c - (NCH - NP) : NP) : (c * NP) / NCH,
                  NCH >= NP ? (c >= NCH - NP ? c - (NCH - NP) + 1 : NP) : ((c + 1) * NP) / NCH);
      __builtin_amdgcn_sched_barrier(0);
    }
    lds_barrier();
    __builtin_amdgcn_sched_barrier(0);
#pragma unroll
    for (int c = 0; c < NCH; ++c) {
      const int s = c / (FM * FN), i = (c / FN) % FM, j = c % FN;
      acc[i][j] = __builtin_amdgcn_mfma_f32_32x32x2f32(af_hi[s][i], bf_hi[s][j], acc[i][j], 0, 0, 0);
      if (c % (FM * FN) == 0) read_kstep(af_lo, bf_lo, buf ^ 1, 0, s);
      __builtin_amdgcn_sched_barrier(0);
    }
  };
  if (kt0 < kt1) {
    load_tiles(ra0, rb0, kt0);
    if constexpr (PF == 2) load_tiles(ra1, rb1, kt0 + 1);
    if constexpr (SEED) {
#pragma unroll
      for (int i = 0; i < FM; ++i)
#pragma unroll
        for (int j = 0; j < FN; ++j) {
          const int col = n0 + wn * TN + j * 32 + li;
#pragma unroll
          for (int r = 0; r < 16; ++r) {
            const float v = g.seed[max(seed_row[i][r], 0ll) * g.ld_seed + min(col, g.N - 1)];
            acc[i][j][r] = (seed_row[i][r] >= 0 && col < g.N) ? v : 0.f;
          }
        }
    }
    store_tiles(ra0, rb0, 0, kt0);
  }
  lds_barrier();
  GEMM_STAMP(1);
  if (kt0 < kt1) {
    read_half(af_lo, bf_lo, 0, 0);
    if constexpr (PF == 1) {
      for (int kt = kt0; kt < kt1; ++kt) step(ra0, rb0, ra0, rb0, kt, (kt - kt0) & 1);
    } else {
      for (int kt = kt0; kt < kt1; kt += 2) {
        step(ra0, rb0, ra1, rb1, kt, 0);
        if (kt + 1 < kt1) step(ra1, rb1, ra0, rb0, kt + 1, 1);
      }
    }
  }

  GEMM_STAMP(2);
  const bool stats = g.stats != nullptr && !partial;
  const bool has_rd = !partial && g.rowdiv != nullptr;
  const int act = g.act;
  float* C = partial ? g.part + static_cast<long long>(blockIdx.z) * g.M * g.N : g.C + batch * g.sc;
  const int ldc = partial ? g.N : g.ldc;
  const bool vec_ok = (ldc & 3) == 0 && (reinterpret_cast<uintptr_t>(C) & 15) == 0;
  double cs[4] = {0.0, 0.0, 0.0, 0.0}, css[4] = {0.0, 0.0, 0.0, 0.0};
#pragma unroll
  for (int pass = 0; pass < BM / CR; ++pass) {
#pragma unroll
    for (int i = 0; i < FM; ++i) {
      const int rbase = wm * TM + i * 32 - pass * CR;
      if (rbase < 0 || rbase >= CR) continue;
#pragma unroll
      for (int j = 0; j < FN; ++j)
#pragma unroll
        for (int r = 0; r < 16; ++r) Cs[rbase + (r & 3) + 8 * (r >> 2) + 4 * lk][wn * TN + j * 32 + li] = acc[i][j][r];
    }
    lds_barrier();
    GEMM_STAMP(4);
#pragma unroll
    for (int it = 0; it < CR / RPI; ++it) {
      const int lrow = it * RPI + rsub;
      const int row = m0 + pass * CR + lrow;
      if (row < g.M && gcol < g.N) {
        const float4 t = *reinterpret_cast<const float4*>(&Cs[lrow][c4]);
        float v[4] = {t.x, t.y, t.z, t.w};
        if (has_rd) {
          const float rd = rdv[pass * (CR / RPI) + it];
#pragma unroll
          for (int e = 0; e < 4; ++e) v[e] = v[e] / rd;
        }
        if (!partial) {
#pragma unroll
          for (int e = 0; e < 4; ++e) {
            const float u = v[e] + bv[e];
            const float neg = act == 2 ? 0.1f * u : 0.f;
            v[e] = (act != 0 && !(u > 0.f)) ? neg : u;
          }
        }
        float* dst = C + static_cast<long long>(row) * ldc + gcol;
        if (vec_ok && gcol + 3 < g.N) {
          *reinterpret_cast<float4*>(dst) = make_float4(v[0], v[1], v[2], v[3]);
        } else {
#pragma unroll
          for (int e = 0; e < 4; ++e)
            if (gcol + e < g.N) dst[e] = v[e];
        }
        if (stats) {
#pragma unroll
          for (int e = 0; e < 4; ++e) {
            cs[e] += v[e];
            css[e] += static_cast<double>(v[e]) * v[e];
          }
        }
      }
    }
    GEMM_STAMP(5);
    lds_barrier();
  }
  if (stats) {
#pragma unroll
    for (int e = 0; e < 4; ++e) {
      stat_red[rsub * BN + c4 + e][0][0] = cs[e];
      stat_red[rsub * BN + c4 + e][0][1] = css[e];
    }
    lds_barrier();
    for (int cl = tid; cl < BN; cl += 256) {
      const int col = n0 + cl;
      if (col >= g.N) continue;
      double a = 0.0, b = 0.0;
#pragma unroll
      for (int w = 0; w < RPI; ++w) {
        a += stat_red[w * BN + cl][0][0];
        b += stat_red[w * BN + cl][0][1];
      }
      g.stats[(static_cast<long long>(tile_y) * 2 + 0) * g.N + col] = a;
      g.stats[(static_cast<long long>(tile_y) * 2 + 1) * g.N + col] = b;
    }
  }
  GEMM_STAMP(3);
}

__device__ __forceinline__ void gemm_small_body(const dim3 blockIdx, const GemmArgs& g, float (*red)[32][33]) {
  const int tid = threadIdx.x, lane = tid & 63, wave = tid >> 6;
  const int li = lane & 31, lk = lane >> 5;
  const int m0 = blockIdx.y * 32, n0 = blockIdx.x * 32;
  const int kq = g.K / 4;
  const int kbeg = wave * kq;
  const int row = min(m0 + li, g.M - 1);
  const int col = n0 + li;
  const bool col_ok = col < g.ldb;
  const float* arow = g.A + static_cast<long long>(row) * g.lda;
  f32x16 acc;
#pragma unroll
  for (int r = 0; r < 16; ++r) acc[r] = 0.f;
  for (int c = 0; c < kq; c += 32) {
    float a[16], b[16];
    const int kb = kbeg + c + lk * 16;
#pragma unroll
    for (int q = 0; q < 4; ++q) {
      float4 v = make_float4(0.f, 0.f, 0.f, 0.f);
      if (c + lk * 16 + 4 * q < kq) v = *reinterpret_cast<const float4*>(arow + kb + 4 * q);
      a[4 * q] = v.x; a[4 * q + 1] = v.y; a[4 * q + 2] = v.z; a[4 * q + 3] = v.w;
    }
#pragma unroll
    for (int t = 0; t < 16; ++t)
      b[t] = (col_ok && c + lk * 16 + t < kq) ? g.B[static_cast<long long>(kb + t) * g.ldb + col] : 0.f;
#pragma unroll
    for (int t = 0; t < 16; ++t) acc = __builtin_amdgcn_mfma_f32_32x32x2f32(a[t], b[t], acc, 0, 0, 0);
  }
#pragma unroll
  for (int r = 0; r < 16; ++r) red[wave][(r & 3) + 8 * (r >> 2) + 4 * lk][li] = acc[r];
  __syncthreads();
#pragma unroll
  for (int q = 0; q < 4; ++q) {
    const int e = tid + 256 * q, rr = e >> 5, cc = e & 31;
    const int orow = m0 + rr, ocol = n0 + cc;
    if (orow < g.M && ocol < g.N) {
      float v = ((red[0][rr][cc] + red[1][rr][cc]) + red[2][rr][cc]) + red[3][rr][cc];
      if (g.bias) v += g.bias[ocol];
      g.C[static_cast<long long>(orow) * g.ldc + ocol] = apply_act(v, g.act);
    }
  }
// ... 261 lines not shown
__device__ __forceinline__ void splitk_reduce_kernel_body(const dim3 blockIdx, const dim3 gridDim, GemmArgs g, int batches) {
  (void)blockIdx; (void)gridDim;
  const long long total = static_cast<long long>(batches) * g.M * g.N;
  for (long long i = blockIdx.x * static_cast<long long>(blockDim.x) + threadIdx.x; i < total;
       i += static_cast<long long>(gridDim.x) * blockDim.x) {
    const int n = static_cast<int>(i % g.N);
    const int m = static_cast<int>((i / g.N) % g.M);
    const int b = static_cast<int>(i / (static_cast<long long>(g.M) * g.N));
    const float* p = g.part + (static_cast<long long>(b) * g.splits) * g.M * g.N +
                     static_cast<long long>(m) * g.N + n;
    float v = 0.f;
    for (int s = 0; s < g.splits; ++s) v += p[static_cast<long long>(s) * g.M * g.N];
    if (g.rowdiv) v = v / g.rowdiv[m];
    if (g.bias) v += g.bias[n];
    g.C[b * g.sc + static_cast<long long>(m) * g.ldc + n] = apply_act(v, g.act);
  }
}


constexpr int kStatRowsPerLane = 8;
inline int stat_rows_per_block(long long n) { return kStatRowsPerLane * (256 / static_cast<int>(n < 256 ? n : 256)); }
__device__ __forceinline__ void splitk_reduce_stats_kernel_body(const dim3 blockIdx, const dim3 gridDim, GemmArgs g, double* stats) {
  (void)blockIdx; (void)gridDim;
  __shared__ double red[2][256];
  const int cw = g.N < 256 ? g.N : 256;
  const int lanes = 256 / cw;
  const int r0 = blockIdx.x * (kStatRowsPerLane * lanes);
  const int r1 = min(g.M, r0 + kStatRowsPerLane * lanes);
  const int col_in = threadIdx.x % cw, rl = threadIdx.x / cw;
  const int col = blockIdx.y * 256 + col_in;
  double s = 0.0, ss = 0.0;
  if (rl < lanes && col < g.N) {
    const float bv = g.bias ? g.bias[col] : 0.f;
    const long long plane = static_cast<long long>(g.M) * g.N;
    float acc[kStatRowsPerLane];
    const float* p[kStatRowsPerLane];
#pragma unroll
    for (int u = 0; u < kStatRowsPerLane; ++u) {
      const int r = min(r0 + rl + u * lanes, g.M - 1);
      p[u] = g.part + static_cast<long long>(r) * g.N + col;
      acc[u] = 0.f;
    }
    for (int k = 0; k < g.splits; ++k) {
#pragma unroll
      for (int u = 0; u < kStatRowsPerLane; ++u) acc[u] += p[u][k * plane];
    }
#pragma unroll
    for (int u = 0; u < kStatRowsPerLane; ++u) {
      const int r = r0 + rl + u * lanes;
      if (r >= r1) break;
      float v = acc[u];
      if (g.rowdiv) v = v / g.rowdiv[r];
      v = apply_act(v + bv, g.act);
      g.C[static_cast<long long>(r) * g.ldc + col] = v;
      const double d = v;
      s += d;
      ss += d * d;
    }
  }
  red[0][threadIdx.x] = s;
  red[1][threadIdx.x] = ss;
  __syncthreads();
  if (threadIdx.x < cw && col < g.N) {
    double a = 0.0, b = 0.0;
    for (int k = 0; k < lanes; ++k) {
      a += red[0][k * cw + threadIdx.x];
      b += red[1][k * cw + threadIdx.x];
    }
    stats[(static_cast<long long>(blockIdx.x) * 2 + 0) * g.N + col] = a;
    stats[(static_cast<long long>(blockIdx.x) * 2 + 1) * g.N + col] = b;
  }
}


thread_local unsigned g_lds_pad = 0;

template <int BM, int BN, int WM, int WN, int BK, int PF = 1>
void launch(const GemmArgs& g, int batches, bool trans_b, hipStream_t st) {
  dim3 grid(ceil_div(g.N, BN), ceil_div(g.M, BM), batches * g.splits);
  constexpr int kMinWaves = BM * BN <= 64 * 64 ? 4 : 1;
  static const int pad_env = [] { const char* v = ::rdm::dev_knob("RDM_GEMM_LDS_PAD"); return v ? atoi(v) : -1; }();
  const unsigned pad = pad_env >= 0 ? static_cast<unsigned>(pad_env) : g_lds_pad;
  if constexpr (BM == 64 && BN == 64 && BK == 32 && PF == 2) {
    if (g.aidx && g.bidx) {
      ::rdm::launch<gemm_kernel_body<BM, BN, WM, WN, BK, true, PF, true>, 256, kMinWaves>(grid, pad, st, g);
      return;
    }
    if (g.aidx) {
      ::rdm::launch<gemm_kernel_body<BM, BN, WM, WN, BK, false, PF, true>, 256, kMinWaves>(grid, pad, st, g);
      return;
    }
    if (g.seed) {
      ::rdm::launch<gemm_kernel_body<BM, BN, WM, WN, BK, false, PF, false, true>, 256, kMinWaves>(grid, pad, st, g);
      return;
    }
  }
  if (trans_b)
    ::rdm::launch<gemm_kernel_body<BM, BN, WM, WN, BK, true, PF>, 256, kMinWaves>(grid, pad, st, g);
  else
    ::rdm::launch<gemm_kernel_body<BM, BN, WM, WN, BK, false, PF>, 256, kMinWaves>(grid, pad, st, g);
}

}

void rdm::gemm_set_lds_pad(unsigned bytes) { g_lds_pad = bytes; }

extern "C" size_t rdm_gemm_workspace_bytes(int64_t m, int64_t n, int batches) {
  const size_t by_shape = static_cast<size_t>(m) * static_cast<size_t>(n) * 16;
  const size_t by_tiles = static_cast<size_t>(1024) * 128 * 128;
  return align_up(std::min(by_shape, by_tiles) * sizeof(float) * static_cast<size_t>(batches > 0 ? batches : 1));
}

namespace {

thread_local int g_last_plan[4] = {0, 0, 0, 0};

enum Tile { T128, T64, T128x32 };

struct GemmPlan {
  bool small = false;
  Tile tile = T64;
  int bm = 64, bn = 64, bk = 32;
  int splits = 1;
  int exp_tile = 0;
  int xcd_tiles = 0;
};

bool small_kernel_ok(long long m, long long n, long long k) {
  return m <= 1536 && k % 16 == 0 && k >= 64 && k <= 1024 && m * n <= 1536 * 512;
}

void set_tile_shape(GemmPlan& p, long long k, bool gathered) {
  p.bm = p.tile == T64 ? 64 : 128;
  p.bn = p.tile == T128 ? 128 : (p.tile == T64 ? 64 : 32);
  p.bk = p.tile == T128 ? 16 : ((p.tile == T64 ? (k >= 48 || gathered) : k >= 32) ? 32 : 16);
}

GemmPlan plan_tiled(const GemmArgs& g, int batches, size_t ws_cap, long long model_cus = 256) {
  const long long m = g.M, n = g.N, k = g.K;
  struct Cand { Tile tile; int bm, bn; double fixed_us, lat_k64_us, mfma_k64_us; int resident; double alpha; };
  static const Cand cands[3] = {{T128, 128, 128, 4.0, 2.6, 3.4, 3, 0.0}, {T64, 64, 64, 1.5, 2.2, 0.86, 4, 0.2},
                                {T128x32, 128, 32, 3.0, 1.3, 0.86, 3, 0.0}};
  static const int split_set[8] = {1, 2, 3, 4, 6, 8, 12, 16};
  GemmPlan p;
  double best = 1e30;
  for (const Cand& c : cands) {
    if (g.aidx && c.tile != T64) continue;
    if (c.tile == T128x32 && n > 64) continue;
    if (c.tile != T128x32 && n <= 32) continue;
    if (c.tile == T128 && n < 128) continue;
    const long long tiles = ceil_div<long long>(m, c.bm) * ceil_div<long long>(n, c.bn) * batches;
    const int max_s = k >= 256 ? static_cast<int>(std::min<long long>(16, k / 128)) : 1;
    for (int sp : split_set) {
      if (sp > max_s) break;
      if (sp > 1 && static_cast<size_t>(m) * n * sp * batches * sizeof(float) > ws_cap) break;
      const long long blocks = tiles * sp;
      const double k_per = static_cast<double>(k) / sp / 64.0;
      const long long per_round = model_cus * c.resident;
      const long long full = blocks / per_round, rem = blocks % per_round;
      auto per_k64 = [&](double r) { return std::max(c.lat_k64_us * (1.0 + c.alpha * (r - 1.0)), c.mfma_k64_us * r); };
      double t = full * (c.fixed_us + k_per * per_k64(c.resident));
      if (rem) t += c.fixed_us + k_per * per_k64(static_cast<double>(ceil_div<long long>(rem, model_cus)));
      if (sp > 1) t += 3.0 + static_cast<double>(m) * n * sp * 8.0 / 1.5e6;
      if (t < best) {
        best = t;
        p.tile = c.tile;
// ... 61 lines not shown
  set_tile_shape(p, k, g.aidx != nullptr);
  static const bool bk16 = ::rdm::dev_knob("RDM_GEMM_BK16") != nullptr;
  if (bk16 && p.tile == T64 && !g.aidx) p.bk = 16;
  if (p.exp_tile) {
    p.bm = p.exp_tile == 5 ? 64 : (p.exp_tile == 7 ? 256 : 128);
    p.bn = (p.exp_tile == 5 || p.exp_tile == 6) ? 128 : 64;
    p.bk = 32;
  }
}
#endif

int launch_plan(const GemmPlan& p, GemmArgs g, int batches, bool trans_b, void* ws, int* stat_blocks, hipStream_t st) {
  const long long m = g.M, n = g.N;
  g_last_plan[0] = p.bm; g_last_plan[1] = p.bn; g_last_plan[2] = p.bk; g_last_plan[3] = p.splits;
  if (g.seed && (p.small || p.exp_tile || p.tile != T64 || p.bk != 32 || p.splits != 1 || batches != 1 || trans_b || g.aidx)) {
    set_error("gemm: seeded accumulators exist for the un-split 64 x 64 x 32 tile only");
    return RDM_ERR_ARG;
  }
  if (p.small) {
    if (stat_blocks) *stat_blocks = 0;
    RDM_DUP_LOOP("gemmsmall")
    ::rdm::launch<gemm_small_entry, 256>(dim3(ceil_div<long long>(n, 32), ceil_div<long long>(m, 32)), 0, st, g);
    return launch_status("gemm_small_kernel");
  }
  g.xcd_tiles = p.xcd_tiles;
  if (p.splits > 1) {
    g.splits = p.splits;
    g.part = static_cast<float*>(ws);
  }
  double* reduce_stats = nullptr;
  if (g.splits > 1) {
    if (batches == 1 && g.N % 4 == 0) reduce_stats = g.stats;
    g.stats = nullptr;
  }
  if (stat_blocks)
    *stat_blocks = g.stats ? static_cast<int>(ceil_div<long long>(m, p.bm))
                           : (reduce_stats ? static_cast<int>(ceil_div<long long>(m, stat_rows_per_block(n))) : 0);
  RDM_DUP_LOOP("gemm") {
#ifdef RDM_DEV_KNOBS
  if (p.exp_tile == 4) launch<128, 64, 2, 2, 32, 2>(g, batches, trans_b, st);
  else if (p.exp_tile == 5) launch<64, 128, 2, 2, 32, 2>(g, batches, trans_b, st);
  else if (p.exp_tile == 6) launch<128, 128, 2, 2, 32, 2>(g, batches, trans_b, st);
  else if (p.exp_tile == 7) launch<256, 64, 4, 1, 32, 2>(g, batches, trans_b, st);
  else
#endif
  switch (p.tile) {
    case T128: launch<128, 128, 2, 2, 16>(g, batches, trans_b, st); break;
    case T64:
      if (p.bk == 32) launch<64, 64, 2, 2, 32, 2>(g, batches, trans_b, st);
      else launch<64, 64, 2, 2, 16>(g, batches, trans_b, st);
      break;
    case T128x32:
      if (p.bk == 32) launch<128, 32, 4, 1, 32, 2>(g, batches, trans_b, st);
      else launch<128, 32, 4, 1, 16>(g, batches, trans_b, st);
      break;
  }
  }
  if (int e = launch_status("gemm_kernel")) return e;
  if (g.splits > 1 && reduce_stats) {
    RDM_DUP_LOOP("splitk")
    ::rdm::launch<splitk_reduce_stats_kernel_body, 256>(dim3(ceil_div<long long>(m, stat_rows_per_block(n)), ceil_div<long long>(n, 256)), 0, st, g, reduce_stats);
    return launch_status("splitk_reduce_stats_kernel");
  }
  if (g.splits > 1) {
    const long long total = static_cast<long long>(batches) * m * n;
    const int blocks = static_cast<int>(std::min<long long>(ceil_div<long long>(total, 256), 2048));
    ::rdm::launch<splitk_reduce_kernel_body, 256>(dim3(blocks), 0, st, g, batches);
    return launch_status("splitk_reduce_kernel");
  }
  return RDM_OK;
}

int gemm_dispatch(const GemmArgs& g, int batches, bool trans_b, void* ws, size_t ws_bytes, int* stat_blocks, hipStream_t st) {
  const size_t ws_cap = ws ? ws_bytes : 0;
  GemmPlan p = plan_gemm(g, batches, trans_b, ws_cap);
#ifdef RDM_DEV_KNOBS
  lab_overrides(p, g, batches, ws_cap);
#endif
  return launch_plan(p, g, batches, trans_b, ws, stat_blocks, st);
}

}

int rdm::gemm_with_stats(const float* a, int64_t lda, const float* b, int64_t ldb, float* c, int64_t ldc, int64_t m,
                         int64_t n, int64_t k, const float* bias, const float* rowdiv, void* ws, size_t ws_bytes,
                         double* gn_partial, int* gn_blocks, void* stream) {
  GemmArgs g;
  g.A = a; g.B = b; g.C = c; g.bias = bias; g.rowdiv = rowdiv;
  g.M = static_cast<int>(m); g.N = static_cast<int>(n); g.K = static_cast<int>(k);
  g.lda = static_cast<int>(lda); g.ldb = static_cast<int>(ldb); g.ldc = static_cast<int>(ldc);
  g.stats = gn_partial;
  return gemm_dispatch(g, 1, false, ws, ws_bytes, gn_blocks, static_cast<hipStream_t>(stream));
}

int rdm::gemm_concat_with_stats(const float* coarse, int64_t ld1, int64_t c1, int64_t n_coarse, const int64_t* idx, int64_t ldi,
                                const float* skip, int64_t ld2, int64_t c2, const float* b, int64_t ldb, float* c, int64_t ldc,
                                int64_t m, int64_t n, int64_t n_need, const float* bias, int act, float* pbuf, size_t pbuf_floats,
                                void* ws, size_t ws_bytes, double* gn_partial, int* gn_blocks, void* stream) {
  if (c1 % 32 != 0 || c2 % 4 != 0 || c2 < 4 || ld1 % 4 != 0 || ld2 % 4 != 0 || ldb % 4 != 0 || m <= 0 ||
      ((reinterpret_cast<uintptr_t>(coarse) | reinterpret_cast<uintptr_t>(skip) | reinterpret_cast<uintptr_t>(b)) & 15) != 0)
    return 1;
  GemmArgs g;
  g.A = coarse; g.B = b; g.C = c; g.bias = bias;
  g.M = static_cast<int>(m); g.N = static_cast<int>(n); g.K = static_cast<int>(c1 + c2);
  g.lda = static_cast<int>(ld1); g.ldb = static_cast<int>(ldb); g.ldc = static_cast<int>(ldc);
  g.act = act; g.stats = gn_partial;
  g.A2 = skip; g.aidx = idx; g.lda2 = static_cast<int>(ld2); g.ldi = static_cast<int>(ldi); g.c1 = static_cast<int>(c1);
  g.n_coarse = static_cast<int>(n_coarse);
  hipStream_t st = static_cast<hipStream_t>(stream);
  const size_t ws_cap = ws ? ws_bytes : 0;
  GemmPlan p = plan_gemm(g, 1, false, ws_cap);
#ifdef RDM_DEV_KNOBS
  lab_overrides(p, g, 1, ws_cap);
#endif
  if (p.splits == 1) n = n_need;
  g.N = static_cast<int>(n);
  const int64_t ldp = (n + 3) / 4 * 4;
  const bool seeded = p.splits == 1 && p.tile == T64 && p.bk == 32 && p.exp_tile == 0 && n_coarse > 0 && n_coarse < m &&
                      pbuf && static_cast<size_t>(n_coarse) * ldp <= pbuf_floats && (reinterpret_cast<uintptr_t>(pbuf) & 15) == 0;
  if (!seeded) return launch_plan(p, g, 1, false, ws, gn_blocks, st);
  GemmArgs gp;
  gp.A = coarse; gp.B = b; gp.C = pbuf;
  gp.M = static_cast<int>(n_coarse); gp.N = static_cast<int>(n); gp.K = static_cast<int>(c1);
  gp.lda = static_cast<int>(ld1); gp.ldb = static_cast<int>(ldb); gp.ldc = static_cast<int>(ldp);
  const GemmPlan pp = plan_tiled(gp, 1, 0);
  if (int e = launch_plan(pp, gp, 1, false, nullptr, nullptr, st)) return e;
  GemmArgs gs;
  gs.A = skip; gs.B = b + c1 * ldb; gs.C = c; gs.bias = bias;
  gs.M = static_cast<int>(m); gs.N = static_cast<int>(n); gs.K = static_cast<int>(c2);
  gs.lda = static_cast<int>(ld2); gs.ldb = static_cast<int>(ldb); gs.ldc = static_cast<int>(ldc);
  gs.act = act; gs.stats = gn_partial;
  gs.seed = pbuf; gs.ld_seed = static_cast<int>(ldp); gs.sidx = idx; gs.ldsi = static_cast<int>(ldi); gs.n_seed = static_cast<int>(n_coarse);
  GemmPlan ps;
  ps.tile = T64; ps.splits = 1;
  set_tile_shape(ps, c2, true);
  return launch_plan(ps, gs, 1, false, nullptr, gn_blocks, st);
}

int rdm::gemm_pair(const float* a0, int64_t lda0, const float* b0, int64_t ldb0, float* c0, int64_t ldc0, int64_t m0, int64_t n0,
                   int64_t k0, const float* bias0, const float* a1, int64_t lda1, const float* b1, int64_t ldb1, float* c1,
                   int64_t ldc1, int64_t m1, int64_t n1, int64_t k1, const float* bias1, void* ws, size_t ws_bytes, void* stream) {
  bool small = m0 > 0 && m1 > 0 && small_kernel_ok(m0, n0, k0) && small_kernel_ok(m1, n1, k1) && lda0 % 4 == 0 && lda1 % 4 == 0 &&
               ldb0 % 4 == 0 && ldb1 % 4 == 0 && ((reinterpret_cast<uintptr_t>(a0) | reinterpret_cast<uintptr_t>(a1)) & 15) == 0;
#ifdef RDM_DEV_KNOBS
  small = small && !lab_tune_skips_small();
#endif
  if (small) {
    GemmArgs g[2];
    const float* A[2] = {a0, a1}; const float* B[2] = {b0, b1}; float* C[2] = {c0, c1}; const float* bias[2] = {bias0, bias1};
    const int64_t M[2] = {m0, m1}, N[2] = {n0, n1}, K[2] = {k0, k1}, LA[2] = {lda0, lda1}, LB[2] = {ldb0, ldb1}, LC[2] = {ldc0, ldc1};
    for (int i = 0; i < 2; ++i) {
      g[i].A = A[i]; g[i].B = B[i]; g[i].C = C[i]; g[i].bias = bias[i];
      g[i].M = static_cast<int>(M[i]); g[i].N = static_cast<int>(N[i]); g[i].K = static_cast<int>(K[i]);
      g[i].lda = static_cast<int>(LA[i]); g[i].ldb = static_cast<int>(LB[i]); g[i].ldc = static_cast<int>(LC[i]);
    }
    const long long gx = ceil_div<long long>(std::max(n0, n1), 32), gy = ceil_div<long long>(std::max(m0, m1), 32);
    ::rdm::launch<gemm_small_pair_entry, 256>(dim3(gx, gy, 2), 0, static_cast<hipStream_t>(stream), g[0], g[1]);
    return launch_status("gemm_small_pair_kernel");
  }
  if (m0 > 0)
    if (int e = rdm_gemm(a0, lda0, 0, b0, ldb0, 0, 0, c0, ldc0, 0, m0, n0, k0, 1, bias0, nullptr, 0, ws, ws_bytes, stream)) return e;
  if (m1 > 0) return rdm_gemm(a1, lda1, 0, b1, ldb1, 0, 0, c1, ldc1, 0, m1, n1, k1, 1, bias1, nullptr, 0, ws, ws_bytes, stream);
  return RDM_OK;
}

extern "C" int rdm_gemm_last_plan(int* out4_host) {
  using namespace rdm;
  RDM_REQUIRE(out4_host, "rdm_gemm_last_plan: null pointer");
  for (int i = 0; i < 4; ++i) out4_host[i] = g_last_plan[i];
  return RDM_OK;
}

extern "C" int rdm_gemm(const float* a, int64_t lda, int64_t stride_a, const float* b, int64_t ldb,
                        int64_t stride_b, int trans_b, float* c, int64_t ldc, int64_t stride_c,
                        int64_t m, int64_t n, int64_t k, int batches, const float* bias,
// ... 201 lines not shown
```

rdmnet_amd/csrc/internal.h:

```cpp
#pragma once
#include <cstddef>
#include <cstdint>

namespace rdm {

int gemm_with_stats(const float* a, int64_t lda, const float* b, int64_t ldb, float* c, int64_t ldc, int64_t m,
                    int64_t n, int64_t k, const float* bias, const float* rowdiv, void* ws, size_t ws_bytes,
                    double* gn_partial, int* gn_blocks, void* stream);

void gemm_set_lds_pad(unsigned bytes);
int gemm_concat_with_stats(const float* coarse, int64_t ld1, int64_t c1, int64_t n_coarse, const int64_t* idx, int64_t ldi,
                           const float* skip, int64_t ld2, int64_t c2, const float* b, int64_t ldb, float* c, int64_t ldc,
                           int64_t m, int64_t n, int64_t n_need, const float* bias, int act, float* pbuf, size_t pbuf_floats,
                           void* ws, size_t ws_bytes, double* gn_partial, int* gn_blocks, void* stream);
int decoder_stage_cols(const float* coarse, int64_t n_coarse, int64_t c1, int64_t ld1, const int64_t* idx, int64_t ldi,
                       const float* skip, int64_t c2, int64_t ld2, int64_t m, const float* w, int64_t ldw, const float* bias,
                       int64_t n, int64_t n_need, int groups, const float* gamma, const float* beta, float eps, int act,
                       float* lin_out, int64_t ld_lin, float* y, int64_t ldy, void* ws, size_t ws_bytes, void* stream);

int gemm_pair(const float* a0, int64_t lda0, const float* b0, int64_t ldb0, float* c0, int64_t ldc0, int64_t m0, int64_t n0,
              int64_t k0, const float* bias0, const float* a1, int64_t lda1, const float* b1, int64_t ldb1, float* c1,
              int64_t ldc1, int64_t m1, int64_t n1, int64_t k1, const float* bias1, void* ws, size_t ws_bytes, void* stream);

inline int64_t gemm_stats_max_blocks(int64_t m) { return (m + 7) / 8 + 1; }

int grid_subsample_mode(const float* points, int64_t n_points, const int64_t* lengths, int batch, float voxel_size,
                        float* out_points, int64_t* out_lengths, void* ws, size_t ws_bytes, void* stream, int mode);

int group_norm_finish(const double* partial, int nblk, const float* x, int64_t n, int64_t c, int64_t ldx, int groups,
                      const float* gamma, const float* beta, float eps, const float* residual, int64_t ldr, int act,
                      float* y, int64_t ldy, uint8_t* positive, void* ws, size_t ws_bytes, void* stream, int form = 0);

int gather_rows_multi(int n, const void* const* x, const int64_t* n_src, const int64_t* words, const int64_t* ldx,
                      const int64_t* const* idx, const int64_t* m, void* const* y, const int64_t* ldy, void* stream);

int radius_grid_build_multi(int n, const float* const* s_points, const int64_t* n_s, const int64_t* const* s_lengths, int batch,
                            const float* radius, void* const* grid_ws, const size_t* grid_ws_bytes, void* stream);

int radius_grid_build_trivial(const float* s_points, int64_t n_s, const int64_t* s_lengths, int batch, void* grid_ws,
                              size_t grid_ws_bytes, void* stream);

int compact_indices_pair(const uint8_t* keep, int64_t n_ref, int64_t n, int32_t* order, int32_t* counts,
                         const int32_t* mirror_src, int32_t* mirror_dst, int mirror_words, void* stream);

int gather_max_ordered(const float* x, int64_t n_s, int64_t c, int64_t ldx, const int64_t* idx, int64_t m, int64_t h, int64_t ldi,
                       const int32_t* width, float* y, int64_t ldy, const float* order_records, int i32, void* stream);
int kpconv_gather_impl(const float* q_points, int64_t m, const float* s_points, int64_t n_s, const float* s_feats, int64_t c,
                       int64_t ldf, const uint8_t* s_positive, const int64_t* idx, int64_t h, int64_t ldi, const int32_t* width,
                       const float* kernel_points, float sigma, float* wf, int64_t ldw, float* nn, const float* order_records,
                       int i32, void* stream, int form = 0);
bool kpconv_tile_gather_applies(int64_t c, int64_t h, bool has_order);
int kpconv_tile_gather(const float* q_points, int64_t m, const float* s_points, int64_t n_s, const float* s_feats, int64_t c,
                       int64_t ldf, const uint8_t* s_positive, const int64_t* idx, int64_t h, int64_t ldi, const int32_t* width,
                       const float* kernel_points, float sigma, float* wf, int64_t ldw, float* nn, const float* order_records,
                       int i32, void* stream);
int kpconv_fused_impl(const float* q_points, int64_t m, const float* s_points, int64_t n_s, const float* s_feats, int64_t c,
                      int64_t ldf, const uint8_t* s_positive, const int64_t* idx, int64_t h, int64_t ldi, const int32_t* width,
                      const float* kernel_points, float sigma, const float* w_packed, const float* bias, int64_t c_out, float* out,
                      int64_t ldo, double* gn_partial, const float* order_records, int form, int i32, void* stream);

size_t radius_redo_queue_bytes();
void radius_redo_queue_reset(void* queue);
int radius_grid_query_deferred(void* grid_ws, size_t grid_ws_bytes, int64_t n_s, const float* q_points, int64_t n_q,
                               const int64_t* q_lengths, int batch, float radius, int width, int64_t* out_idx,
                               int32_t* out_counts, int32_t* out_max, int32_t* status, unsigned char* redo_flags, void* queue,
                               int i32, void* stream);
int radius_redo_flush(void* queue, void* stream);

}
```

rdmnet_amd/csrc/kpconv.hip:

```cpp
#include "../../include/rdmnet_hip.h"
#include "common.h"
#include "internal.h"
#include "lockstep.h"

namespace {

using namespace rdm;

typedef float f32x4 __attribute__((ext_vector_type(4)));

constexpr int kKP = 15;
constexpr int kMaxH = 128;
constexpr int kWaves = 4;

struct KpArgs {
  const float* q_points;
  const float* s_points;
  const float* s_feats;
  const unsigned char* s_pos;
  const int64_t* idx;
  int i32;
  const float* kp;
  const int32_t* width;
  const float4* order;
  int units_per_block;
  int split;
  int xcd_remap;
  float* wf;
  float* nn;
  int M, Ns, H, C;
  int ldf, ldi, ldw;
  float sigma;
};

template <int VEC, int U, int SPLIT, int PF>
__device__ __forceinline__ void kpconv_gather_kernel_body(const dim3 blockIdx, const dim3 gridDim, KpArgs a) {
  (void)blockIdx; (void)gridDim;
  __shared__ float4 nb[kWaves][kMaxH];
  const int wave = threadIdx.x >> 6, lane = threadIdx.x & 63;
  const int split = SPLIT > 0 ? SPLIT : a.split;
  const int total_units = a.M * split;
  const int qpb = a.units_per_block;
  const int nblk = gridDim.x;
  int blk = blockIdx.x;
  if ((qpb > kWaves || a.xcd_remap) && nblk >= 16) {
    const int q = nblk / 8, rr = nblk % 8, xcd = blk % 8, within = blk / 8;
    blk = (xcd < rr ? xcd * (q + 1) : rr * (q + 1) + (xcd - rr) * q) + within;
  }
  const int g = lane >> 4, j = lane & 15;
  const float kx = j < kKP ? a.kp[3 * j] : 0.f, ky = j < kKP ? a.kp[3 * j + 1] : 0.f,
              kz = j < kKP ? a.kp[3 * j + 2] : 0.f;
  const float inv_sigma = 1.0f / a.sigma;
  for (int u0 = wave; u0 < qpb; u0 += kWaves) {
  const int unit = blk * qpb + u0;
  if (unit >= total_units) break;
  const int slice = unit % split;
  const int m = a.order ? __float_as_int(a.order[unit / split].w) : unit / split;
  int H = a.H;
  if (a.width) H = min(H, *a.width);
  const int c_base = slice * (16 * VEC * U);

  const float qx = a.q_points[3 * m], qy = a.q_points[3 * m + 1], qz = a.q_points[3 * m + 2];
  int positives = 0;
  f32x4 acc[VEC * U];
#pragma unroll
  for (int t = 0; t < VEC * U; ++t) acc[t] = f32x4{0.f, 0.f, 0.f, 0.f};
  for (int hc = 0; hc < H; hc += kMaxH) {
  const int Hc = min(H - hc, kMaxH);
  int Hq = 0;
  for (int hb = 0; hb < Hc; hb += 64) {
    const int h = hb + lane;
    const int64_t id = h < Hc ? ld_index(a.idx, static_cast<int64_t>(m) * a.ldi + hc + h, a.i32) : -1;
    const bool real = id >= 0 && id < a.Ns;
    const unsigned long long rm = __builtin_amdgcn_ballot_w64(real);
    if (rm) Hq = hb + 64 - __builtin_clzll(rm);
    float4 v;
    if (real) {
      v.x = a.s_points[3 * id] - qx;
      v.y = a.s_points[3 * id + 1] - qy;
      v.z = a.s_points[3 * id + 2] - qz;
      v.w = __int_as_float(static_cast<int>(id));
      positives += a.s_pos[id];
    } else {
      v.x = 1.0e6f - qx;
      v.y = 1.0e6f - qy;
      v.z = 1.0e6f - qz;
      v.w = __int_as_float(-1);
    }
    if (h < Hc) nb[wave][h] = v;
  }
  __builtin_amdgcn_fence(__ATOMIC_SEQ_CST, "wavefront");
  __builtin_amdgcn_wave_barrier();

  for (int h0 = 0; h0 < Hq; h0 += 4 * PF) {
    float w[PF];
    float f[PF][U][VEC];
#pragma unroll
    for (int p = 0; p < PF; ++p) {
      const int h = h0 + 4 * p + g;
      int id = -1;
      w[p] = 0.f;
      if (h < Hq) {
        const float4 v = nb[wave][h];
        id = __float_as_int(v.w);
        const float dx = v.x - kx, dy = v.y - ky, dz = v.z - kz;
        const float d2 = (dx * dx + dy * dy) + dz * dz;
        w[p] = fmaxf(0.f, 1.f - __builtin_amdgcn_sqrtf(d2) * inv_sigma);
        if (j >= kKP || id < 0) w[p] = 0.f;
      }
      const float* row = a.s_feats + static_cast<int64_t>(id < 0 ? 0 : id) * a.ldf + c_base + VEC * j;
#pragma unroll
      for (int u = 0; u < U; ++u) {
        if (id >= 0) {
          if (VEC == 4) {
            const float4 t = *reinterpret_cast<const float4*>(row + 16 * VEC * u);
            f[p][u][0] = t.x; f[p][u][1] = t.y; f[p][u][2] = t.z; f[p][u][VEC - 1] = t.w;
          } else if (VEC == 2) {
            const float2 t = *reinterpret_cast<const float2*>(row + 16 * VEC * u);
            f[p][u][0] = t.x; f[p][u][VEC - 1] = t.y;
          } else {
            f[p][u][0] = row[16 * VEC * u];
          }
        } else {
#pragma unroll
          for (int e = 0; e < VEC; ++e) f[p][u][e] = 0.f;
        }
      }
    }
#pragma unroll
    for (int p = 0; p < PF; ++p)
#pragma unroll
      for (int u = 0; u < U; ++u)
#pragma unroll
        for (int e = 0; e < VEC; ++e)
          acc[u * VEC + e] = __builtin_amdgcn_mfma_f32_16x16x4f32(w[p], f[p][u][e], acc[u * VEC + e], 0, 0, 0);
  }
  __builtin_amdgcn_fence(__ATOMIC_SEQ_CST, "wavefront");
  __builtin_amdgcn_wave_barrier();
  }
  positives = wave_sum_i(positives);

  float* out = a.wf + static_cast<int64_t>(m) * a.ldw + c_base;
#pragma unroll
  for (int r = 0; r < 4; ++r) {
    const int k = 4 * g + r;
    if (k >= kKP) continue;
#pragma unroll
    for (int u = 0; u < U; ++u) {
      float* p = out + k * a.C + 16 * VEC * u + VEC * j;
      if (VEC == 4) {
        *reinterpret_cast<float4*>(p) = make_float4(acc[u * 4 + 0][r], acc[u * 4 + 1][r],
                                                    acc[u * 4 + 2][r], acc[u * 4 + 3][r]);
      } else if (VEC == 2) {
        *reinterpret_cast<float2*>(p) = make_float2(acc[u * 2 + 0][r], acc[u * 2 + 1][r]);
      } else {
        p[0] = acc[u][r];
      }
    }
  }
  if (lane == 0 && slice == 0) a.nn[m] = static_cast<float>(positives > 1 ? positives : 1);
  }
}


__device__ __forceinline__ void kpconv_gather_c1_kernel_body(const dim3 blockIdx, const dim3 gridDim, KpArgs a) {
  (void)blockIdx; (void)gridDim;
  __shared__ float4 nb[kWaves][kMaxH];
  const int wave = threadIdx.x >> 6, lane = threadIdx.x & 63;
  const int mu = blockIdx.x * kWaves + wave;
  if (mu >= a.M) return;
  const int m = a.order ? __float_as_int(a.order[mu].w) : mu;
  int H = a.H;
  if (a.width) H = min(H, *a.width);
  const float qx = a.q_points[3 * m], qy = a.q_points[3 * m + 1], qz = a.q_points[3 * m + 2];
  const int g = lane >> 4, j = lane & 15;
  const float kx = j < kKP ? a.kp[3 * j] : 0.f, ky = j < kKP ? a.kp[3 * j + 1] : 0.f,
              kz = j < kKP ? a.kp[3 * j + 2] : 0.f;
  const float inv_sigma = 1.0f / a.sigma;
  int positives = 0;
  float acc = 0.f;
  for (int hc = 0; hc < H; hc += kMaxH) {
    const int Hc = min(H - hc, kMaxH);
    int Hq = 0;
    for (int hb = 0; hb < Hc; hb += 64) {
      const int h = hb + lane;
      const int64_t id = h < Hc ? ld_index(a.idx, static_cast<int64_t>(m) * a.ldi + hc + h, a.i32) : -1;
      float4 v = make_float4(0.f, 0.f, 0.f, 0.f);
      const unsigned long long rm = __builtin_amdgcn_ballot_w64(id >= 0 && id < a.Ns);
      if (rm) Hq = hb + 64 - __builtin_clzll(rm);
      if (id >= 0 && id < a.Ns) {
        v.x = a.s_points[3 * id] - qx;
        v.y = a.s_points[3 * id + 1] - qy;
        v.z = a.s_points[3 * id + 2] - qz;
        v.w = a.s_feats[id * a.ldf];
        positives += a.s_pos[id];
      }
      if (h < Hc) nb[wave][h] = v;
    }
    __builtin_amdgcn_fence(__ATOMIC_SEQ_CST, "wavefront");
    __builtin_amdgcn_wave_barrier();
    for (int h = g; h < Hq; h += 4) {
      const float4 v = nb[wave][h];
      const float dx = v.x - kx, dy = v.y - ky, dz = v.z - kz;
      const float d2 = (dx * dx + dy * dy) + dz * dz;
      acc += fmaxf(0.f, 1.f - __builtin_amdgcn_sqrtf(d2) * inv_sigma) * v.w;
    }
    __builtin_amdgcn_fence(__ATOMIC_SEQ_CST, "wavefront");
    __builtin_amdgcn_wave_barrier();
  }
  positives = wave_sum_i(positives);
  acc += __shfl_xor(acc, 16, 64);
  acc += __shfl_xor(acc, 32, 64);
  float* out = a.wf + static_cast<int64_t>(m) * a.ldw;
  if (g == 0) {
    if (j < kKP) out[j] = acc;
    else {
      for (int k = kKP; k < a.ldw; ++k) out[k] = 0.f;
      a.nn[m] = static_cast<float>(positives > 1 ? positives : 1);
    }
  }
}


__device__ __forceinline__ void row_positive_kernel_body(const dim3 blockIdx, const dim3 gridDim, const float* x, int n, int c, int ld, unsigned char* out) {
  (void)blockIdx; (void)gridDim;
  const int row = blockIdx.x * (blockDim.x >> 6) + (threadIdx.x >> 6);
  if (row >= n) return;
  const int lane = threadIdx.x & 63;
  float s = 0.f;
  for (int i = lane; i < c; i += 64) s += x[static_cast<int64_t>(row) * ld + i];
  s = wave_sum(s);
  if (lane == 0) out[row] = s > 0.f ? 1 : 0;
}


}

extern "C" int rdm_row_positive(const float* x, int64_t n, int64_t c, int64_t ld, uint8_t* out,
                                void* stream) {
  using namespace rdm;
  RDM_REQUIRE(x && out && n >= 0 && c > 0, "rdm_row_positive: bad arguments");
  if (n == 0) return RDM_OK;
  ::rdm::launch<row_positive_kernel_body, 256>(dim3(ceil_div<int64_t>(n, 4)), 0, static_cast<hipStream_t>(stream), x, static_cast<int>(n), static_cast<int>(c),
                     static_cast<int>(ld), out);
  return launch_status("row_positive_kernel");
}

namespace {
bool tile_gather_pays(int64_t c, int64_t m) {
  (void)c; (void)m;
  return false;
}
}

int rdm::kpconv_gather_impl(const float* q_points, int64_t m, const float* s_points, int64_t n_s, const float* s_feats, int64_t c,
                            int64_t ldf, const uint8_t* s_positive, const int64_t* idx, int64_t h, int64_t ldi, const int32_t* width,
                            const float* kernel_points, float sigma, float* wf, int64_t ldw, float* nn, const float* order_records,
                            int i32, void* stream, int form) {
  using namespace rdm;
  RDM_REQUIRE(q_points && s_points && s_feats && s_positive && idx && kernel_points && wf && nn,
              "rdm_kpconv_gather: null pointer");
  RDM_REQUIRE(m >= 0 && n_s > 0 && h > 0, "rdm_kpconv_gather: bad sizes (h=%lld)", (long long)h);
  RDM_REQUIRE(c == 1 || c % 32 == 0, "rdm_kpconv_gather: unsupported channel count %lld (1 or a multiple of 32)", (long long)c);
  RDM_REQUIRE(ldw >= kKP * c && (c == 1 || (ldf % 4 == 0 && ldw % 4 == 0)),
              "rdm_kpconv_gather: ldw/ldf must be padded");
  if (m == 0) return RDM_OK;
  if (form != 1 && kpconv_tile_gather_applies(c, h, order_records != nullptr) && (form == 2 || tile_gather_pays(c, m)))
    return kpconv_tile_gather(q_points, m, s_points, n_s, s_feats, c, ldf, s_positive, idx, h, ldi, width, kernel_points, sigma, wf,
                              ldw, nn, order_records, i32, stream);
  KpArgs a;
  a.q_points = q_points; a.s_points = s_points; a.s_feats = s_feats; a.s_pos = s_positive;
  a.idx = idx; a.i32 = i32 ? 1 : 0; a.kp = kernel_points; a.width = width; a.wf = wf; a.nn = nn;
  a.order = reinterpret_cast<const float4*>(order_records);
  a.M = static_cast<int>(m); a.Ns = static_cast<int>(n_s); a.H = static_cast<int>(h);
  a.C = static_cast<int>(c); a.ldf = static_cast<int>(ldf); a.ldi = static_cast<int>(ldi);
  a.ldw = static_cast<int>(ldw); a.sigma = sigma; a.split = 1;
  static const bool xcd_env = ::rdm::dev_knob("RDM_GATHER_XCD") != nullptr;
  a.xcd_remap = (xcd_env && order_records) ? 1 : 0;
  hipStream_t st = static_cast<hipStream_t>(stream);
  auto grid = [&](int split) {
    a.units_per_block = kWaves;
    return dim3(static_cast<unsigned>(ceil_div<int64_t>(m * split, a.units_per_block)));
  };
  RDM_DUP_LOOP("gather")
  switch (c) {
    case 1: ::rdm::launch<kpconv_gather_c1_kernel_body, 64 * kWaves>(dim3(ceil_div<int64_t>(m, kWaves)), 0, st, a); break;
    case 32: ::rdm::launch<kpconv_gather_kernel_body<2, 1, 1, 4>, 64 * kWaves>(grid(1), 0, st, a); break;
    case 64: ::rdm::launch<kpconv_gather_kernel_body<4, 1, 1, 4>, 64 * kWaves>(grid(1), 0, st, a); break;
    case 128: ::rdm::launch<kpconv_gather_kernel_body<4, 1, 2, 4>, 64 * kWaves>(grid(2), 0, st, a); break;
    case 256: ::rdm::launch<kpconv_gather_kernel_body<4, 1, 4, 4>, 64 * kWaves>(grid(4), 0, st, a); break;
    case 512: ::rdm::launch<kpconv_gather_kernel_body<4, 2, 4, 2>, 64 * kWaves>(grid(4), 0, st, a); break;
    default:
      a.split = static_cast<int>(c / 32);
      ::rdm::launch<kpconv_gather_kernel_body<2, 1, 0, 4>, 64 * kWaves>(grid(a.split), 0, st, a);
      break;
  }
  return launch_status("kpconv_gather_kernel");
}

extern "C" int rdm_kpconv_gather_ordered(const float* q_points, int64_t m, const float* s_points, int64_t n_s,
                                         const float* s_feats, int64_t c, int64_t ldf, const uint8_t* s_positive,
                                         const int64_t* idx, int64_t h, int64_t ldi, const int32_t* width,
                                         const float* kernel_points, float sigma, float* wf, int64_t ldw,
                                         float* nn, const float* order_records, void* stream) {
  return rdm::kpconv_gather_impl(q_points, m, s_points, n_s, s_feats, c, ldf, s_positive, idx, h, ldi, width, kernel_points, sigma,
                                 wf, ldw, nn, order_records, 0, stream);
}

extern "C" int rdm_kpconv_gather_form(const float* q_points, int64_t m, const float* s_points, int64_t n_s,
                                      const float* s_feats, int64_t c, int64_t ldf, const uint8_t* s_positive,
                                      const int64_t* idx, int64_t h, int64_t ldi, const int32_t* width,
                                      const float* kernel_points, float sigma, float* wf, int64_t ldw,
                                      float* nn, const float* order_records, int form, void* stream) {
  RDM_REQUIRE(form >= 0 && form <= 2, "rdm_kpconv_gather_form: form must be 0, 1 or 2");
  return rdm::kpconv_gather_impl(q_points, m, s_points, n_s, s_feats, c, ldf, s_positive, idx, h, ldi, width, kernel_points, sigma,
                                 wf, ldw, nn, order_records, 0, stream, form);
}

extern "C" int rdm_kpconv_gather(const float* q_points, int64_t m, const float* s_points, int64_t n_s,
                                 const float* s_feats, int64_t c, int64_t ldf, const uint8_t* s_positive,
                                 const int64_t* idx, int64_t h, int64_t ldi, const int32_t* width,
                                 const float* kernel_points, float sigma, float* wf, int64_t ldw,
                                 float* nn, void* stream) {
  return rdm_kpconv_gather_ordered(q_points, m, s_points, n_s, s_feats, c, ldf, s_positive, idx, h, ldi, width, kernel_points,
                                   sigma, wf, ldw, nn, nullptr, stream);
}
```

rdmnet_amd/engine.py:

```python
import ctypes

import numpy as np
import torch

from . import _lib, config, weights


class EngineConfig(ctypes.Structure):
    _fields_ = [('num_stages', ctypes.c_int), ('kernel_size', ctypes.c_int), ('group_norm', ctypes.c_int),
                ('init_voxel_size', ctypes.c_float), ('init_radius', ctypes.c_float), ('init_sigma', ctypes.c_float),
                ('neighbor_limits', ctypes.c_int * 5), ('out_dim', ctypes.c_int), ('num_heads', ctypes.c_int),
                ('num_layers', ctypes.c_int), ('num_layers2', ctypes.c_int), ('vote_mlp_layers', ctypes.c_int),
                ('vote_limit', ctypes.c_float * 3), ('nms_radius', ctypes.c_float), ('points_in_patch', ctypes.c_int),
                ('num_correspondences', ctypes.c_int), ('dual_normalization', ctypes.c_int),
                ('sinkhorn_iterations', ctypes.c_int), ('acceptance_radius', ctypes.c_float),
                ('correspondence_threshold', ctypes.c_int), ('num_refinement_steps', ctypes.c_int),
                ('use_vote', ctypes.c_int), ('attention_bf16', ctypes.c_int),
                ('arena_bytes', ctypes.c_size_t)]


class EngineResult(ctypes.Structure):
    _fields_ = [('transform', ctypes.c_float * 16), ('n_correspondences', ctypes.c_int32),
                ('n_hypotheses', ctypes.c_int32), ('best_hypothesis', ctypes.c_int32),
                ('n_ref_nodes', ctypes.c_int64), ('n_src_nodes', ctypes.c_int64),
# ... 29 lines not shown


_DTYPES = {0: torch.float32, 1: torch.int64, 2: torch.uint8, 3: torch.int32}
_ESIZE = {0: 4, 1: 8, 2: 1, 3: 4}
POINT_LEVELS = {'input': 0, 'fine': 1, 'coarse': 2}


def make_config(cfg, arena_bytes=0):
    c = EngineConfig()
    b, t, fm = cfg.backbone, cfg.thdroformer, cfg.fine_matching
    c.num_stages, c.kernel_size, c.group_norm = b.num_stages, b.kernel_size, b.group_norm
    c.init_voxel_size, c.init_radius, c.init_sigma = b.init_voxel_size, b.init_radius, b.init_sigma
    c.neighbor_limits = (ctypes.c_int * 5)(*[int(x) for x in cfg.neighbor_limits])
    c.out_dim, c.num_heads, c.num_layers, c.num_layers2 = t.output_dim, t.num_heads, t.num_layers, t.num_layers2
    c.vote_mlp_layers = len(cfg.Vote.MLPS)
    c.vote_limit = (ctypes.c_float * 3)(*[float(x) for x in cfg.Vote.MAX_TRANSLATE_RANGE])
    c.nms_radius = cfg.Vote.NMS_radius
    c.points_in_patch = cfg.model.num_points_in_patch
    c.num_correspondences = cfg.coarse_matching.num_correspondences
    c.dual_normalization = int(cfg.coarse_matching.dual_normalization)
    c.sinkhorn_iterations = cfg.model.num_sinkhorn_iterations
    c.acceptance_radius, c.correspondence_threshold = fm.acceptance_radius, fm.correspondence_threshold
    c.num_refinement_steps = fm.num_refinement_steps
    c.use_vote = int(bool(cfg.Vote.model_use_vote and cfg.Vote.inference_use_vote))
    c.attention_bf16 = int(bool(getattr(cfg.thdroformer, 'attention_bf16', False)))
    c.arena_bytes = arena_bytes
    return c


class Engine:

    def __init__(self, cfg, state, device=None, arena_bytes=0, share_with=None):
        if not torch.cuda.is_available():
            raise RuntimeError('rdmnet_amd.engine needs a GPU (no CPU fallback)')
        self.L = _lib.lib()
        self.device = torch.device('cuda', torch.cuda.current_device()) if device is None else torch.device(device)
        self.cfg = cfg
        self._h = ctypes.c_void_p()
        topk = config.topk_fractions(cfg)
        fm = config.fine_matching_options(cfg)
        with torch.cuda.device(self.device):
            c = make_config(cfg, arena_bytes)
            _lib.check(self.L.rdm_engine_create(ctypes.byref(c), ctypes.byref(self._h)), 'rdm_engine_create')
            if topk is not None:
                fr = (ctypes.c_double * len(topk))(*topk)
                _lib.check(self.L.rdm_engine_set_attention_topk(self._h, len(topk), fr), 'rdm_engine_set_attention_topk')
            if fm is not None:
                opt = _lib.FineMatchingOptions.of(**fm)
                _lib.check(self.L.rdm_engine_set_fine_matching(self._h, ctypes.byref(opt)), 'rdm_engine_set_fine_matching')
            if share_with is not None:
                _lib.check(self.L.rdm_engine_share_params(self._h, share_with._h), 'rdm_engine_share_params')
            for name, shape in ({} if share_with is not None else weights.schema(cfg)).items():
                v = state[name]
                v = v.detach().cpu().numpy() if isinstance(v, torch.Tensor) else np.asarray(v)
                if tuple(v.shape) != tuple(shape):
                    raise RuntimeError(f'size mismatch for {name}: {tuple(v.shape)} vs {tuple(shape)}')
                v = np.ascontiguousarray(v, dtype=np.float32)
                shp = (ctypes.c_int64 * max(len(shape), 1))(*shape)
                _lib.check(self.L.rdm_engine_set_param(self._h, name.encode(), v.ctypes.data, ctypes.addressof(shp),
                                                       len(shape)), 'rdm_engine_set_param')
            if share_with is None:
                _lib.check(self.L.rdm_engine_finalize(self._h), 'rdm_engine_finalize')
        self.result = EngineResult()
        self._export_cache = {}
        self._ran, self._prepared = None, []

    def __del__(self):
        h = getattr(self, '_h', None)
        if h is not None and h.value:
            try:
                self.L.rdm_engine_destroy(h)
            except Exception:
                pass
            h.value = None

    def set_wait(self, sleep_us=0):
        _lib.check(self.L.rdm_engine_set_wait(self._h, int(sleep_us)), 'rdm_engine_set_wait')

    def set_pairs_in_flight(self, n):
        _lib.check(self.L.rdm_engine_set_pairs_in_flight(self._h, int(n)), 'rdm_engine_set_pairs_in_flight')

    def set_overlap(self, mode=1):
        _lib.check(self.L.rdm_engine_set_overlap(self._h, int(mode)), 'rdm_engine_set_overlap')

    def reserve(self, arena_bytes):
        self.clear_pending()
        _lib.check(self.L.rdm_engine_reserve(self._h, int(arena_bytes)), 'rdm_engine_reserve')

    def enable_profile(self, enable=True):
        _lib.check(self.L.rdm_engine_enable_profile(self._h, int(enable)), 'rdm_engine_enable_profile')

    def kpconv_profile(self):
        buf = (KpconvProfile * 16)()
        n = self.L.rdm_engine_get_profile(self._h, ctypes.addressof(buf), 16)
        out = []
        for p in buf[:max(n, 0)]:
            gather = p.m * p.h * (8 + 12 + 4 * p.c_in)
            total = gather + 4 * p.m * p.c_out + (p.m * p.h * (8 + 4 * p.pooled_channels) if p.pooled_channels else 0)
            out.append({'m': p.m, 'h': p.h, 'cin': p.c_in, 'cout': p.c_out, 'bytes': total, 'gather_bytes': gather,
                        'gather_ms': p.gather_ms, 'total_ms': p.total_ms, 'pooled': int(p.pooled_channels), 'fused': int(p.fused)})
        return out

    def keep_taps(self, enable=True):
        self.clear_pending()
        _lib.check(self.L.rdm_engine_keep_taps(self._h, int(enable)), 'rdm_engine_keep_taps')

    @staticmethod
    def _held(ref, src):
        return (ref, src, ref._version, src._version)

    @staticmethod
    def _is_held(held, ref, src):
        r, s, vr, vs = held
        same = lambda a, b: a is b or (a.data_ptr() == b.data_ptr() and a.shape == b.shape and a.stride() == b.stride())
        return same(r, ref) and same(s, src) and ref._version == vr and src._version == vs

    def clear_pending(self):
        self._ran = None
        self._prepared = []

    def run(self, ref_points, src_points):
        assert ref_points.is_cuda and ref_points.dtype == torch.float32 and ref_points.is_contiguous()
        assert src_points.is_cuda and src_points.dtype == torch.float32 and src_points.is_contiguous()
        ran = getattr(self, '_ran', None)
        if ran is not None:
            self._ran = None
            if self._is_held(ran, ref_points, src_points):
                return self.result
        prepared = getattr(self, '_prepared', None)
        if prepared:
            k, held = prepared[0]
            if self._is_held(held, ref_points, src_points):
                prepared.pop(0)
                return self.forward_batched(k)
            self._prepared = []
        _lib.check(self.L.rdm_engine_run(self._h, ref_points.data_ptr(), ref_points.shape[0], src_points.data_ptr(),
                                         src_points.shape[0], ctypes.byref(self.result), _lib.stream_ptr()),
                   'rdm_engine_run')
        return self.result

    def collate_batch(self, pairs):
        n = len(pairs)
        for r, s in pairs:
            assert r.is_cuda and r.dtype == torch.float32 and r.is_contiguous() and s.is_cuda and s.dtype == torch.float32 and s.is_contiguous()
        P, I = ctypes.c_void_p * n, ctypes.c_int64 * n
        rp, sp = P(*[r.data_ptr() for r, _ in pairs]), P(*[s.data_ptr() for _, s in pairs])
        rn, sn = I(*[r.shape[0] for r, _ in pairs]), I(*[s.shape[0] for _, s in pairs])
        self.clear_pending()
        _lib.check(self.L.rdm_engine_collate_batch(self._h, n, rp, rn, sp, sn, _lib.stream_ptr()), 'rdm_engine_collate_batch')
        self._prepared = [(k, self._held(r, s)) for k, (r, s) in enumerate(pairs)]
        return n

    @staticmethod
    def run_lockstep(engines, pairs, collate_batched=True):
        n = len(pairs)
        assert 1 <= n <= len(engines)
        for r, s in pairs:
            assert r.is_cuda and r.dtype == torch.float32 and r.is_contiguous() and s.is_cuda and s.dtype == torch.float32 and s.is_contiguous()
        P, I = ctypes.c_void_p * n, ctypes.c_int64 * n
        for e in engines[:n]:
            e.clear_pending()
        hs = P(*[e._h.value if hasattr(e._h, 'value') else e._h for e in engines[:n]])
        rp, sp = P(*[r.data_ptr() for r, _ in pairs]), P(*[s.data_ptr() for _, s in pairs])
        rn, sn = I(*[r.shape[0] for r, _ in pairs]), I(*[s.shape[0] for _, s in pairs])
        res = P(*[ctypes.addressof(e.result) for e in engines[:n]])
        _lib.check(engines[0].L.rdm_engine_run_lockstep(hs, n, rp, rn, sp, sn, res, int(bool(collate_batched)), _lib.stream_ptr()), 'rdm_engine_run_lockstep')
# ... 293 lines not shown
```

Before: 619.6.

## Skip zero kernel-point k-tiles in KPConv GEMM via influence masks and row reordering

The gather kernel now records, for each query row, which of the 15 kernel points have any nonzero influence weight. A new ordering kernel ranks the rows so that rows with similar masks share 64-row tiles, and builds a per-tile OR mask. The KPConv GEMM gains a ZSKIP variant that builds a per-tile list of live k-tiles in LDS, loads only those, and scatters output rows back through the permutation. This avoids multiply work on k-slices that are entirely zero, at the cost of an extra ordering kernel, the permuted gathers, and forgoing the tile-gather path whenever masks are produced.

```diff
diff --git a/include/rdmnet_hip.h b/include/rdmnet_hip.h
--- a/include/rdmnet_hip.h
+++ b/include/rdmnet_hip.h
@@ -157,6 +157,16 @@
                               const int64_t* idx, int64_t h, int64_t ldi, const int32_t* width,
                               const float* kernel_points, float sigma, float* wf, int64_t ldw, float* nn,
                               const float* order_records, int form, void* stream);
+int rdm_kpconv_gather_mask(const float* q_points, int64_t m, const float* s_points, int64_t n_s,
+                           const float* s_feats, int64_t c, int64_t ldf, const uint8_t* s_positive,
+                           const int64_t* idx, int64_t h, int64_t ldi, const int32_t* width,
+                           const float* kernel_points, float sigma, float* wf, int64_t ldw, float* nn,
+                           const float* order_records, int32_t* mask, void* stream);
+int rdm_kpconv_tile_order(const int32_t* mask, int64_t m, int64_t* perm, int32_t* tile_mask, void* stream);
+int rdm_kpconv_contract(const float* wf, int64_t ldw, const float* w, int64_t ldb, float* out, int64_t ldo, int64_t m,
+                        int64_t c_in, int64_t c_out, const float* bias, const float* rowdiv, const int64_t* perm,
+                        const int32_t* tile_mask, int splits, void* ws, size_t ws_bytes, double* gn_partial,
+                        int* gn_blocks_host, void* stream);
 int rdm_row_positive(const float* x, int64_t n, int64_t c, int64_t ld, uint8_t* out, void* stream);
 
 size_t rdm_group_norm_workspace_bytes(int64_t n, int64_t c);
@@ -399,6 +409,7 @@
 int rdm_engine_set_wait(rdm_engine* e, int sleep_us);
 int rdm_engine_set_pairs_in_flight(rdm_engine* e, int n);
 int rdm_engine_set_overlap(rdm_engine* e, int mode);
+int rdm_engine_set_kpconv_zero_tiles(rdm_engine* e, int enable);
 int rdm_engine_set_attention_topk(rdm_engine* e, int n_layers, const double* fracs);
 int rdm_engine_set_fine_matching(rdm_engine* e, const rdm_fine_matching_options* options);
 int rdm_engine_enable_profile(rdm_engine* e, int enable);
diff --git a/rdmnet_amd/_lib.py b/rdmnet_amd/_lib.py
--- a/rdmnet_amd/_lib.py
+++ b/rdmnet_amd/_lib.py
@@ -85,6 +85,11 @@
                                           c_i64, c_void, c_void, c_f32, c_void, c_i64, c_void, c_void, c_void]),
     'rdm_kpconv_gather_form': (c_int, [c_void, c_i64, c_void, c_i64, c_void, c_i64, c_i64, c_void, c_void, c_i64,
                                        c_i64, c_void, c_void, c_f32, c_void, c_i64, c_void, c_void, c_int, c_void]),
+    'rdm_kpconv_gather_mask': (c_int, [c_void, c_i64, c_void, c_i64, c_void, c_i64, c_i64, c_void, c_void, c_i64,
+                                       c_i64, c_void, c_void, c_f32, c_void, c_i64, c_void, c_void, c_void, c_void]),
+    'rdm_kpconv_tile_order': (c_int, [c_void, c_i64, c_void, c_void, c_void]),
+    'rdm_kpconv_contract': (c_int, [c_void, c_i64, c_void, c_i64, c_void, c_i64, c_i64, c_i64, c_i64, c_void, c_void, c_void,
+                                    c_void, c_int, c_void, c_size, c_void, c_void, c_void]),
     'rdm_kpconv_fused_enabled': (c_int, []),
     'rdm_kpconv_fused_supported': (c_int, [c_i64, c_i64]),
     'rdm_kpconv_fused_partial_rows': (c_i64, [c_i64, c_i64]),
@@ -230,6 +235,7 @@
     'rdm_engine_set_wait': (c_int, [c_void, c_int]),
     'rdm_engine_set_pairs_in_flight': (c_int, [c_void, c_int]),
     'rdm_engine_set_overlap': (c_int, [c_void, c_int]),
+    'rdm_engine_set_kpconv_zero_tiles': (c_int, [c_void, c_int]),
     'rdm_engine_set_attention_topk': (c_int, [c_void, c_int, c_void]),
     'rdm_engine_set_fine_matching': (c_int, [c_void, c_void]),
     'rdm_engine_enable_profile': (c_int, [c_void, c_int]),
diff --git a/rdmnet_amd/csrc/engine.hip b/rdmnet_amd/csrc/engine.hip
--- a/rdmnet_amd/csrc/engine.hip
+++ b/rdmnet_amd/csrc/engine.hip
@@ -107,6 +107,7 @@
   int pairs_in_flight = 1;
   int overlap_mode = 1;
   hipStream_t side = nullptr;
+  bool kpconv_zero_tiles = true;
   std::map<hipStream_t, bool> side_ok;
   std::vector<PairPyramid> batch;
   std::vector<int64_t> batch_n_ref, batch_n_src;
@@ -371,19 +372,34 @@
   ENG_ALLOC(wf.p);
   float* nn = e->alloc<float>(q.n > 0 ? q.n : 1);
   ENG_ALLOC(nn);
+  const size_t gemm_ws = rdm_gemm_workspace_bytes(q.n, W.out, 1);
+  static const bool dense_knob = ::rdm::dev_knob("RDM_KPCONV_DENSE") != nullptr;
+  const bool skip = e->kpconv_zero_tiles && !dense_knob && cin % 32 == 0 && W.kpad == kdim && kpconv_tile_order_applies(q.n) &&
+                    kpconv_contract_skips(q.n, cin, W.out, gemm_ws);
+  int32_t *mask = nullptr, *tile_mask = nullptr;
+  int64_t* perm = nullptr;
+  if (skip) {
+    mask = e->alloc<int32_t>(q.n);
+    perm = e->alloc<int64_t>(q.n);
+    tile_mask = e->alloc<int32_t>((q.n + 63) / 64);
+    ENG_ALLOC(mask); ENG_ALLOC(perm); ENG_ALLOC(tile_mask);
+  }
   if (prof) ENG_CHECK(layer_event(e, 3 * li, r.st));
   ENG_CHECK(kpconv_gather_impl(q.pts, q.n, s.pts, s.n, x.p, cin, x.ld, x_pos, t.idx, t.width, t.stride(), t.flags,
-                               vecp(r, name + ".kernel_points"), sigma, wf.p, wf.ld, nn, order, i32, r.st));
+                               vecp(r, name + ".kernel_points"), sigma, wf.p, wf.ld, nn, order, i32, r.st, 0, mask, tile_mask));
   if (prof) ENG_CHECK(layer_event(e, 3 * li + 1, r.st));
+  if (skip) {
+    ENG_CHECK(kpconv_tile_order(mask, q.n, perm, tile_mask, true, r.st));
+    tap(r, (name + ".tile_mask").c_str(), tile_mask, (q.n + 63) / 64, 1, 1, 3);
+  }
   Mat conv = e->mat(q.n, W.out);
   ENG_ALLOC(conv.p);
-  const size_t gemm_ws = rdm_gemm_workspace_bytes(q.n, W.out, 1);
   const size_t stat_bytes = align_up(static_cast<size_t>(gemm_stats_max_blocks(q.n)) * 2 * W.out * sizeof(double));
   RDM_REQUIRE(gemm_ws + stat_bytes + rdm_group_norm_workspace_bytes(q.n, W.out) <= r.ws_bytes, "rdm_engine: scratch too small");
   double* gn_partial = reinterpret_cast<double*>(static_cast<char*>(r.ws) + gemm_ws);
   int gn_blocks = 0;
   ENG_CHECK(gemm_with_stats(wf.p, wf.ld, W.b, W.ldb, conv.p, conv.ld, q.n, W.out, W.kpad, W.bias, nn, r.ws, gemm_ws,
-                            gn_partial, &gn_blocks, r.st));
+                            gn_partial, &gn_blocks, r.st, perm, tile_mask, cin));
   if (pool_src) {
     *pool_out = e->mat(q.n, pool_src->cols);
     ENG_ALLOC(pool_out->p);
@@ -950,6 +966,12 @@
   return RDM_OK;
 }
 
+extern "C" int rdm_engine_set_kpconv_zero_tiles(rdm_engine* e, int enable) {
+  RDM_REQUIRE(e, "rdm_engine_set_kpconv_zero_tiles: null engine");
+  e->kpconv_zero_tiles = enable != 0;
+  return RDM_OK;
+}
+
 extern "C" int rdm_engine_get_profile(rdm_engine* e, rdm_kpconv_profile* out, int cap) {
   RDM_REQUIRE(e && out && cap >= 0, "rdm_engine_get_profile: bad arguments");
   const int n = std::min<int>(cap, static_cast<int>(e->prof.size()));
diff --git a/rdmnet_amd/csrc/gemm.hip b/rdmnet_amd/csrc/gemm.hip
--- a/rdmnet_amd/csrc/gemm.hip
+++ b/rdmnet_amd/csrc/gemm.hip
@@ -35,6 +35,8 @@
   const int64_t* sidx = nullptr;
   int ld_seed = 0, ldsi = 0, n_seed = 0;
   int xcd_tiles = 0;
+  const int32_t* tmask = nullptr;
+  int kp_tiles = 0;
 #ifdef RDM_GEMM_TIMING
   unsigned long long* clk = nullptr;
 #endif
@@ -51,9 +53,11 @@
   return v;
 }
 
-template <int BM, int BN, int WM, int WN, int BK, bool TRANS_B, int PF, bool CAT = false, bool SEED = false>
+constexpr int kSkipListMax = 256;
+template <int BM, int BN, int WM, int WN, int BK, bool TRANS_B, int PF, bool CAT = false, bool SEED = false, bool ZSKIP = false>
 __device__ __forceinline__ void gemm_kernel_body(const dim3 blockIdx, const dim3 gridDim, GemmArgs g) {
   (void)blockIdx; (void)gridDim;
+  static_assert(!ZSKIP || (CAT && !TRANS_B && !SEED && PF == 2), "skipped k-tiles: the row-gathered 32-deep form only");
   constexpr int TM = BM / WM, TN = BN / WN, FM = TM / 32, FN = TN / 32;
   static_assert(WM * WN == 4 && TM % 32 == 0 && TN % 32 == 0, "bad tile");
   static_assert(!SEED || (!CAT && !TRANS_B), "seeded accumulators: plain operands only");
@@ -90,6 +94,29 @@
   const int ktiles = (g.K + BK - 1) / BK;
   const int per = (ktiles + g.splits - 1) / g.splits;
   const int kt0 = split * per, kt1 = min(ktiles, kt0 + per);
+  int nlist = 0;
+  [[maybe_unused]] const unsigned short* klist_p = nullptr;
+  if constexpr (ZSKIP) {
+    __shared__ unsigned short klist[kSkipListMax];
+    __shared__ int wcount[4];
+    const unsigned tm = static_cast<unsigned>(g.tmask[tile_y]);
+    const int t = kt0 + tid;
+    const bool on = t < kt1 && ((tm >> (t / g.kp_tiles)) & 1u) != 0;
+    const unsigned long long bl = __builtin_amdgcn_ballot_w64(on);
+    if (lane == 0) wcount[wave] = __builtin_popcountll(bl);
+    lds_barrier();
+    int before = 0;
+#pragma unroll
+    for (int w = 0; w < 4; ++w) {
+      before += w < wave ? wcount[w] : 0;
+      nlist += wcount[w];
+    }
+    nlist = __builtin_amdgcn_readfirstlane(nlist);
+    if (on) klist[before + __builtin_popcountll(bl & ((1ull << lane) - 1ull))] = static_cast<unsigned short>(t);
+    lds_barrier();
+    klist_p = klist;
+  }
+  [[maybe_unused]] auto listed = [&](int p) { return __builtin_amdgcn_readfirstlane(static_cast<int>(klist_p[min(p, nlist - 1)])); };
 
   constexpr int A_N4 = BM * BK / 4;
   constexpr int A_V = (A_N4 + 255) / 256;
@@ -138,7 +165,7 @@
   }
 
   auto load_tiles = [&](float4 (&ra)[A_V], float4 (&rb)[B_V], int kt, int p0 = 0, int p1 = 1 << 20) {
-    const int k0 = min(kt, kt1 - 1) * BK;
+    const int k0 = (ZSKIP ? kt : min(kt, kt1 - 1)) * BK;
 #pragma unroll
     for (int i = 0; i < A_V; ++i) {
       if (i < p0 || i >= p1) continue;
@@ -146,6 +173,8 @@
       const int row = idx / KC4, kc = (idx % KC4) * 4;
       if constexpr (CAT && TRANS_B) {
         ra[i] = *reinterpret_cast<const float4*>(A + max(cat_row[i], 0ll) * g.lda + min(k0 + kc, g.K - 4));
+      } else if constexpr (ZSKIP) {
+        ra[i] = *reinterpret_cast<const float4*>(A + max(cat_row[i], 0ll) * g.lda + (k0 + kc));
       } else if constexpr (CAT) {
         const float* src = k0 < g.c1 ? A + max(cat_row[i], 0ll) * g.lda + (k0 + kc)
                                      : g.A2 + static_cast<long long>(min(m0 + row, g.M - 1)) * g.lda2 + min(k0 - g.c1 + kc, g.K - g.c1 - 4);
@@ -173,7 +202,7 @@
   };
   auto masked = [](const float4& v, bool ok) { return make_float4(ok ? v.x : 0.f, ok ? v.y : 0.f, ok ? v.z : 0.f, ok ? v.w : 0.f); };
   auto store_tiles = [&](const float4 (&ra)[A_V], const float4 (&rb)[B_V], int buf, int kt, int p0 = 0, int p1 = 1 << 20) {
-    const int k0 = min(kt, kt1 - 1) * BK;
+    const int k0 = (ZSKIP ? kt : min(kt, kt1 - 1)) * BK;
 #pragma unroll
     for (int i = 0; i < A_V; ++i) {
       if (i < p0 || i >= p1) continue;
@@ -226,6 +255,15 @@
     for (int e = 0; e < 4; ++e) bv[e] = gcol + e < g.N ? g.bias[gcol + e] : 0.f;
 #pragma unroll
   for (int q = 0; q < BM / RPI; ++q) rdv[q] = (!partial && g.rowdiv) ? g.rowdiv[min(m0 + q * RPI + rsub, g.M - 1)] : 1.f;
+  int out_row[ZSKIP ? BM / RPI : 1];
+  if constexpr (ZSKIP) {
+#pragma unroll
+    for (int q = 0; q < BM / RPI; ++q) {
+      const int r = m0 + q * RPI + rsub;
+      const long long id = g.aidx[static_cast<long long>(min(r, g.M - 1)) * g.ldi];
+      out_row[q] = (r < g.M && id >= 0 && id < g.M) ? static_cast<int>(id) : -1;
+    }
+  }
 
   const int lk = lane >> 5, li = lane & 31;
   f32x16 acc[FM][FN];
@@ -259,14 +297,17 @@
     for (int s = 0; s < HS; ++s) read_kstep(af, bf, buf, kbase, s);
   };
   constexpr int NCH = HS * FM * FN, NP = A_V + B_V;
+  [[maybe_unused]] int zs = 0, zl = 0;
   auto step = [&](auto& fa, auto& fb, const auto& na, const auto& nb, int kt, int buf) {
+    [[maybe_unused]] int zn = 0;
+    if constexpr (ZSKIP) zn = listed(kt + PF + 1);
 #pragma unroll
     for (int c = 0; c < NCH; ++c) {
       const int s = c / (FM * FN), i = (c / FN) % FM, j = c % FN;
       acc[i][j] = __builtin_amdgcn_mfma_f32_32x32x2f32(af_lo[s][i], bf_lo[s][j], acc[i][j], 0, 0, 0);
       if (c % (FM * FN) == 0) read_kstep(af_hi, bf_hi, buf, HK, s);
-      load_tiles(fa, fb, kt + PF, NCH >= NP ? (c < NP ? c : NP) : (c * NP) / NCH, NCH >= NP ? (c < NP ? c + 1 : NP) : ((c + 1) * NP) / NCH);
-      store_tiles(na, nb, buf ^ 1, kt + 1, NCH >= NP ? (c >= NCH - NP ? c - (NCH - NP) : NP) : (c * NP) / NCH,
+      load_tiles(fa, fb, ZSKIP ? zl : kt + PF, NCH >= NP ? (c < NP ? c : NP) : (c * NP) / NCH, NCH >= NP ? (c < NP ? c + 1 : NP) : ((c + 1) * NP) / NCH);
+      store_tiles(na, nb, buf ^ 1, ZSKIP ? zs : kt + 1, NCH >= NP ? (c >= NCH - NP ? c - (NCH - NP) : NP) : (c * NP) / NCH,
                   NCH >= NP ? (c >= NCH - NP ? c - (NCH - NP) + 1 : NP) : ((c + 1) * NP) / NCH);
       __builtin_amdgcn_sched_barrier(0);
     }
@@ -279,10 +320,16 @@
       if (c % (FM * FN) == 0) read_kstep(af_lo, bf_lo, buf ^ 1, 0, s);
       __builtin_amdgcn_sched_barrier(0);
     }
+    if constexpr (ZSKIP) {
+      zs = zl;
+      zl = zn;
+    }
   };
-  if (kt0 < kt1) {
-    load_tiles(ra0, rb0, kt0);
-    if constexpr (PF == 2) load_tiles(ra1, rb1, kt0 + 1);
+  const int kb = ZSKIP ? 0 : kt0, ke = ZSKIP ? nlist : kt1;
+  auto tile_at = [&](int p) { if constexpr (ZSKIP) return listed(p); else return p; };
+  if (kb < ke) {
+    load_tiles(ra0, rb0, tile_at(kb));
+    if constexpr (PF == 2) load_tiles(ra1, rb1, tile_at(kb + 1));
     if constexpr (SEED) {
 #pragma unroll
       for (int i = 0; i < FM; ++i)
@@ -296,18 +343,22 @@
           }
         }
     }
-    store_tiles(ra0, rb0, 0, kt0);
+    store_tiles(ra0, rb0, 0, tile_at(kb));
   }
   lds_barrier();
   GEMM_STAMP(1);
-  if (kt0 < kt1) {
+  if (kb < ke) {
     read_half(af_lo, bf_lo, 0, 0);
+    if constexpr (ZSKIP) {
+      zs = listed(1);
+      zl = listed(PF);
+    }
     if constexpr (PF == 1) {
-      for (int kt = kt0; kt < kt1; ++kt) step(ra0, rb0, ra0, rb0, kt, (kt - kt0) & 1);
+      for (int kt = kb; kt < ke; ++kt) step(ra0, rb0, ra0, rb0, kt, (kt - kb) & 1);
     } else {
-      for (int kt = kt0; kt < kt1; kt += 2) {
+      for (int kt = kb; kt < ke; kt += 2) {
         step(ra0, rb0, ra1, rb1, kt, 0);
-        if (kt + 1 < kt1) step(ra1, rb1, ra0, rb0, kt + 1, 1);
+        if (kt + 1 < ke) step(ra1, rb1, ra0, rb0, kt + 1, 1);
       }
     }
   }
@@ -337,7 +388,9 @@
     for (int it = 0; it < CR / RPI; ++it) {
       const int lrow = it * RPI + rsub;
       const int row = m0 + pass * CR + lrow;
-      if (row < g.M && gcol < g.N) {
+      bool row_ok = row < g.M;
+      if constexpr (ZSKIP) row_ok = row_ok && out_row[pass * (CR / RPI) + it] >= 0;
+      if (row_ok && gcol < g.N) {
         const float4 t = *reinterpret_cast<const float4*>(&Cs[lrow][c4]);
         float v[4] = {t.x, t.y, t.z, t.w};
         if (has_rd) {
@@ -353,7 +406,7 @@
             v[e] = (act != 0 && !(u > 0.f)) ? neg : u;
           }
         }
-        float* dst = C + static_cast<long long>(row) * ldc + gcol;
+        float* dst = C + static_cast<long long>(ZSKIP ? out_row[pass * (CR / RPI) + it] : row) * ldc + gcol;
         if (vec_ok && gcol + 3 < g.N) {
           *reinterpret_cast<float4*>(dst) = make_float4(v[0], v[1], v[2], v[3]);
         } else {
@@ -781,6 +834,10 @@
   static const int pad_env = [] { const char* v = ::rdm::dev_knob("RDM_GEMM_LDS_PAD"); return v ? atoi(v) : -1; }();
   const unsigned pad = pad_env >= 0 ? static_cast<unsigned>(pad_env) : g_lds_pad;
   if constexpr (BM == 64 && BN == 64 && BK == 32 && PF == 2) {
+    if (g.tmask) {
+      ::rdm::launch<gemm_kernel_body<BM, BN, WM, WN, BK, false, PF, true, false, true>, 256, kMinWaves>(grid, pad, st, g);
+      return;
+    }
     if (g.aidx && g.bidx) {
       ::rdm::launch<gemm_kernel_body<BM, BN, WM, WN, BK, true, PF, true>, 256, kMinWaves>(grid, pad, st, g);
       return;
@@ -1008,15 +1065,72 @@
 
 }
 
+namespace {
+bool zero_tile_route(const GemmPlan& p, long long k, long long c_in) {
+  if (p.small || p.splits <= 1 || p.tile != T64 || p.bk != 32 || p.exp_tile != 0) return false;
+  if (c_in <= 0 || c_in % 32 != 0 || k != 15 * c_in) return false;
+  return ceil_div<long long>(k / 32, p.splits) <= kSkipListMax;
+}
+}
+
 int rdm::gemm_with_stats(const float* a, int64_t lda, const float* b, int64_t ldb, float* c, int64_t ldc, int64_t m,
                          int64_t n, int64_t k, const float* bias, const float* rowdiv, void* ws, size_t ws_bytes,
-                         double* gn_partial, int* gn_blocks, void* stream) {
+                         double* gn_partial, int* gn_blocks, void* stream, const int64_t* perm, const int32_t* tile_mask,
+                         int64_t c_in, int force_splits) {
   GemmArgs g;
   g.A = a; g.B = b; g.C = c; g.bias = bias; g.rowdiv = rowdiv;
   g.M = static_cast<int>(m); g.N = static_cast<int>(n); g.K = static_cast<int>(k);
   g.lda = static_cast<int>(lda); g.ldb = static_cast<int>(ldb); g.ldc = static_cast<int>(ldc);
   g.stats = gn_partial;
-  return gemm_dispatch(g, 1, false, ws, ws_bytes, gn_blocks, static_cast<hipStream_t>(stream));
+  hipStream_t st = static_cast<hipStream_t>(stream);
+  if (!perm && force_splits <= 0) return gemm_dispatch(g, 1, false, ws, ws_bytes, gn_blocks, st);
+  const size_t ws_cap = ws ? ws_bytes : 0;
+  GemmPlan p = plan_gemm(g, 1, false, ws_cap);
+#ifdef RDM_DEV_KNOBS
+  lab_overrides(p, g, 1, ws_cap);
+#endif
+  if (force_splits > 0) {
+    RDM_REQUIRE(static_cast<size_t>(m) * n * force_splits * sizeof(float) <= ws_cap || force_splits == 1,
+                "gemm: the workspace does not hold %d split-K partials", force_splits);
+    p = GemmPlan();
+    p.tile = T64;
+    p.splits = force_splits;
+    set_tile_shape(p, k, false);
+  }
+  if (perm && tile_mask && zero_tile_route(p, k, c_in)) {
+    g.aidx = perm; g.ldi = 1; g.c1 = g.K; g.n_coarse = g.M;
+    g.tmask = tile_mask; g.kp_tiles = static_cast<int>(c_in / 32);
+  }
+  return launch_plan(p, g, 1, false, ws, gn_blocks, st);
+}
+
+bool rdm::kpconv_contract_skips(int64_t m, int64_t c_in, int64_t c_out, size_t ws_bytes) {
+  static const float one = 1.f;
+  static double stat = 0.0;
+  GemmArgs g;
+  g.M = static_cast<int>(m); g.N = static_cast<int>(c_out); g.K = static_cast<int>(15 * c_in);
+  g.rowdiv = &one; g.stats = &stat;
+  GemmPlan p = plan_gemm(g, 1, false, ws_bytes);
+#ifdef RDM_DEV_KNOBS
+  lab_overrides(p, g, 1, ws_bytes);
+#endif
+  return m > 0 && zero_tile_route(p, 15 * c_in, c_in);
+}
+
+extern "C" int rdm_kpconv_contract(const float* wf, int64_t ldw, const float* w, int64_t ldb, float* out, int64_t ldo, int64_t m,
+                                   int64_t c_in, int64_t c_out, const float* bias, const float* rowdiv, const int64_t* perm,
+                                   const int32_t* tile_mask, int splits, void* ws, size_t ws_bytes, double* gn_partial,
+                                   int* gn_blocks_host, void* stream) {
+  using namespace rdm;
+  RDM_REQUIRE(wf && w && out && m > 0 && c_in > 0 && c_in % 32 == 0 && c_out > 0, "rdm_kpconv_contract: bad arguments");
+  RDM_REQUIRE((perm == nullptr) == (tile_mask == nullptr), "rdm_kpconv_contract: perm and tile_mask come together");
+  RDM_REQUIRE(ldw % 4 == 0 && ldb % 4 == 0 && ldw >= 15 * c_in && splits >= 0 && splits <= 16, "rdm_kpconv_contract: bad layout");
+  RDM_REQUIRE(((reinterpret_cast<uintptr_t>(wf) | reinterpret_cast<uintptr_t>(w)) & 15) == 0, "rdm_kpconv_contract: operands must be 16-byte aligned");
+  int blocks = 0;
+  const int rc = gemm_with_stats(wf, ldw, w, ldb, out, ldo, m, c_out, 15 * c_in, bias, rowdiv, ws, ws_bytes, gn_partial, &blocks, stream,
+                                 perm, tile_mask, c_in, splits);
+  if (gn_blocks_host) *gn_blocks_host = blocks;
+  return rc;
 }
 
 int rdm::gemm_concat_with_stats(const float* coarse, int64_t ld1, int64_t c1, int64_t n_coarse, const int64_t* idx, int64_t ldi,
diff --git a/rdmnet_amd/csrc/internal.h b/rdmnet_amd/csrc/internal.h
--- a/rdmnet_amd/csrc/internal.h
+++ b/rdmnet_amd/csrc/internal.h
@@ -6,7 +6,8 @@
 
 int gemm_with_stats(const float* a, int64_t lda, const float* b, int64_t ldb, float* c, int64_t ldc, int64_t m,
                     int64_t n, int64_t k, const float* bias, const float* rowdiv, void* ws, size_t ws_bytes,
-                    double* gn_partial, int* gn_blocks, void* stream);
+                    double* gn_partial, int* gn_blocks, void* stream, const int64_t* perm = nullptr,
+                    const int32_t* tile_mask = nullptr, int64_t c_in = 0, int force_splits = 0);
 
 void gemm_set_lds_pad(unsigned bytes);
 int gemm_concat_with_stats(const float* coarse, int64_t ld1, int64_t c1, int64_t n_coarse, const int64_t* idx, int64_t ldi,
@@ -48,7 +49,10 @@
 int kpconv_gather_impl(const float* q_points, int64_t m, const float* s_points, int64_t n_s, const float* s_feats, int64_t c,
                        int64_t ldf, const uint8_t* s_positive, const int64_t* idx, int64_t h, int64_t ldi, const int32_t* width,
                        const float* kernel_points, float sigma, float* wf, int64_t ldw, float* nn, const float* order_records,
-                       int i32, void* stream, int form = 0);
+                       int i32, void* stream, int form = 0, int32_t* mask = nullptr, int32_t* tile_mask_clear = nullptr);
+bool kpconv_tile_order_applies(int64_t m);
+int kpconv_tile_order(const int32_t* mask, int64_t m, int64_t* perm, int32_t* tile_mask, bool cleared, void* stream);
+bool kpconv_contract_skips(int64_t m, int64_t c_in, int64_t c_out, size_t ws_bytes);
 bool kpconv_tile_gather_applies(int64_t c, int64_t h, bool has_order);
 int kpconv_tile_gather(const float* q_points, int64_t m, const float* s_points, int64_t n_s, const float* s_feats, int64_t c,
                        int64_t ldf, const uint8_t* s_positive, const int64_t* idx, int64_t h, int64_t ldi, const int32_t* width,
diff --git a/rdmnet_amd/csrc/kpconv.hip b/rdmnet_amd/csrc/kpconv.hip
--- a/rdmnet_amd/csrc/kpconv.hip
+++ b/rdmnet_amd/csrc/kpconv.hip
@@ -28,6 +28,9 @@
   int xcd_remap;
   float* wf;
   float* nn;
+  int32_t* mask;
+  int32_t* tmask_clear;
+  int n_tmask;
   int M, Ns, H, C;
   int ldf, ldi, ldw;
   float sigma;
@@ -62,6 +65,7 @@
 
   const float qx = a.q_points[3 * m], qy = a.q_points[3 * m + 1], qz = a.q_points[3 * m + 2];
   int positives = 0;
+  bool felt = false;
   f32x4 acc[VEC * U];
 #pragma unroll
   for (int t = 0; t < VEC * U; ++t) acc[t] = f32x4{0.f, 0.f, 0.f, 0.f};
@@ -107,6 +111,7 @@
         const float d2 = (dx * dx + dy * dy) + dz * dz;
         w[p] = fmaxf(0.f, 1.f - __builtin_amdgcn_sqrtf(d2) * inv_sigma);
         if (j >= kKP || id < 0) w[p] = 0.f;
+        felt |= w[p] > 0.f;
       }
       const float* row = a.s_feats + static_cast<int64_t>(id < 0 ? 0 : id) * a.ldf + c_base + VEC * j;
 #pragma unroll
@@ -159,6 +164,15 @@
     }
   }
   if (lane == 0 && slice == 0) a.nn[m] = static_cast<float>(positives > 1 ? positives : 1);
+  if (a.mask) {
+    unsigned long long b = __builtin_amdgcn_ballot_w64(felt);
+    b |= b >> 32;
+    b |= b >> 16;
+    if (lane == 0 && slice == 0) {
+      a.mask[m] = static_cast<int32_t>(b & 0x7fffu);
+      if (a.tmask_clear && m < a.n_tmask) a.tmask_clear[m] = 0;
+    }
+  }
   }
 }
 
@@ -233,6 +247,81 @@
   if (lane == 0) out[row] = s > 0.f ? 1 : 0;
 }
 
+constexpr int kOrderMaxRows = 16384;
+constexpr int kOrderRows = 16;
+__device__ __forceinline__ void kpconv_tile_order_kernel_body(const dim3 blockIdx, const dim3 gridDim, const int32_t* mask, int M,
+                                                              int64_t* perm, int32_t* tile_mask) {
+  (void)blockIdx; (void)gridDim;
+  __shared__ __attribute__((aligned(16))) unsigned short keys[kOrderMaxRows];
+  __shared__ int empties[kKP], pos[kKP];
+  const int tid = threadIdx.x, lane = tid & 63;
+  if (tid < kKP) empties[tid] = 0;
+  __syncthreads();
+  int cnt[kKP];
+#pragma unroll
+  for (int k = 0; k < kKP; ++k) cnt[k] = 0;
+  for (int j0 = tid; j0 < M; j0 += 256 * 8) {
+    int mk[8];
+#pragma unroll
+    for (int u = 0; u < 8; ++u) mk[u] = mask[min(j0 + 256 * u, M - 1)];
+#pragma unroll
+    for (int u = 0; u < 8; ++u) {
+      const int j = j0 + 256 * u;
+      if (j >= M) break;
+      keys[j] = static_cast<unsigned short>(mk[u] & 0x7fff);
+#pragma unroll
+      for (int k = 0; k < kKP; ++k) cnt[k] += ((mk[u] >> k) & 1) ^ 1;
+    }
+  }
+#pragma unroll
+  for (int k = 0; k < kKP; ++k) {
+    const int c = wave_sum_i(cnt[k]);
+    if (lane == 0) atomicAdd(&empties[k], c);
+  }
+  __syncthreads();
+  if (tid < kKP) {
+    int before = 0;
+    for (int k = 0; k < kKP; ++k) before += (empties[k] > empties[tid] || (empties[k] == empties[tid] && k < tid)) ? 1 : 0;
+    pos[tid] = kKP - 1 - before;
+  }
+  __syncthreads();
+  int ps[kKP];
+#pragma unroll
+  for (int k = 0; k < kKP; ++k) ps[k] = pos[k];
+  for (int j = tid; j < M; j += 256) {
+    const int mk = keys[j];
+    int key = 0;
+#pragma unroll
+    for (int k = 0; k < kKP; ++k) key |= ((mk >> k) & 1) << ps[k];
+    keys[j] = static_cast<unsigned short>(key);
+  }
+  const int groups = (M + 7) / 8;
+  if (tid < 8 && groups * 8 - 8 + tid >= M) keys[groups * 8 - 8 + tid] = 0xffffu;
+  __syncthreads();
+  const int i = blockIdx.x * kOrderRows + (tid >> 4), part = tid & 15;
+  int rank = 0;
+  if (i < M) {
+    const int ki = keys[i];
+    const uint4* keys8 = reinterpret_cast<const uint4*>(keys);
+    for (int gq = part; gq < groups; gq += 16) {
+      const uint4 v = keys8[gq];
+      const unsigned wds[4] = {v.x, v.y, v.z, v.w};
+      const int ahead = i - gq * 8;
+#pragma unroll
+      for (int e = 0; e < 8; ++e) {
+        const int kj = static_cast<int>((e & 1) ? wds[e >> 1] >> 16 : wds[e >> 1] & 0xffffu);
+        rank += kj < ki + (e < ahead ? 1 : 0) ? 1 : 0;
+      }
+    }
+  }
+#pragma unroll
+  for (int o = 1; o < 16; o <<= 1) rank += __shfl_xor(rank, o, 64);
+  if (i < M && part == 0) {
+    perm[rank] = i;
+    atomicOr(&tile_mask[rank >> 6], mask[i] & 0x7fff);
+  }
+}
+
 
 }
 
@@ -256,7 +345,7 @@
 int rdm::kpconv_gather_impl(const float* q_points, int64_t m, const float* s_points, int64_t n_s, const float* s_feats, int64_t c,
                             int64_t ldf, const uint8_t* s_positive, const int64_t* idx, int64_t h, int64_t ldi, const int32_t* width,
                             const float* kernel_points, float sigma, float* wf, int64_t ldw, float* nn, const float* order_records,
-                            int i32, void* stream, int form) {
+                            int i32, void* stream, int form, int32_t* mask, int32_t* tile_mask_clear) {
   using namespace rdm;
   RDM_REQUIRE(q_points && s_points && s_feats && s_positive && idx && kernel_points && wf && nn,
               "rdm_kpconv_gather: null pointer");
@@ -265,12 +354,14 @@
   RDM_REQUIRE(ldw >= kKP * c && (c == 1 || (ldf % 4 == 0 && ldw % 4 == 0)),
               "rdm_kpconv_gather: ldw/ldf must be padded");
   if (m == 0) return RDM_OK;
-  if (form != 1 && kpconv_tile_gather_applies(c, h, order_records != nullptr) && (form == 2 || tile_gather_pays(c, m)))
+  RDM_REQUIRE(!mask || c % 32 == 0, "rdm_kpconv_gather: the influence mask exists for c a multiple of 32");
+  if (!mask && form != 1 && kpconv_tile_gather_applies(c, h, order_records != nullptr) && (form == 2 || tile_gather_pays(c, m)))
     return kpconv_tile_gather(q_points, m, s_points, n_s, s_feats, c, ldf, s_positive, idx, h, ldi, width, kernel_points, sigma, wf,
                               ldw, nn, order_records, i32, stream);
   KpArgs a;
   a.q_points = q_points; a.s_points = s_points; a.s_feats = s_feats; a.s_pos = s_positive;
   a.idx = idx; a.i32 = i32 ? 1 : 0; a.kp = kernel_points; a.width = width; a.wf = wf; a.nn = nn;
+  a.mask = mask; a.tmask_clear = mask ? tile_mask_clear : nullptr; a.n_tmask = static_cast<int>(ceil_div<int64_t>(m, 64));
   a.order = reinterpret_cast<const float4*>(order_records);
   a.M = static_cast<int>(m); a.Ns = static_cast<int>(n_s); a.H = static_cast<int>(h);
   a.C = static_cast<int>(c); a.ldf = static_cast<int>(ldf); a.ldi = static_cast<int>(ldi);
@@ -298,6 +389,32 @@
   return launch_status("kpconv_gather_kernel");
 }
 
+bool rdm::kpconv_tile_order_applies(int64_t m) { return m > 0 && m <= kOrderMaxRows; }
+int rdm::kpconv_tile_order(const int32_t* mask, int64_t m, int64_t* perm, int32_t* tile_mask, bool cleared, void* stream) {
+  using namespace rdm;
+  RDM_REQUIRE(mask && perm && tile_mask, "rdm_kpconv_tile_order: null pointer");
+  RDM_REQUIRE(kpconv_tile_order_applies(m), "rdm_kpconv_tile_order: 1 to %d rows (m=%lld)", kOrderMaxRows, (long long)m);
+  hipStream_t st = static_cast<hipStream_t>(stream);
+  if (!cleared) fill_words<int32_t>(tile_mask, ceil_div<int64_t>(m, 64), 0, st);
+  RDM_DUP_LOOP("tileorder")
+  ::rdm::launch<kpconv_tile_order_kernel_body, 256>(dim3(static_cast<unsigned>(ceil_div<int64_t>(m, kOrderRows))), 0, st, mask, static_cast<int>(m),
+                                                    perm, tile_mask);
+  return launch_status("kpconv_tile_order_kernel");
+}
+
+extern "C" int rdm_kpconv_tile_order(const int32_t* mask, int64_t m, int64_t* perm, int32_t* tile_mask, void* stream) {
+  return rdm::kpconv_tile_order(mask, m, perm, tile_mask, false, stream);
+}
+
+extern "C" int rdm_kpconv_gather_mask(const float* q_points, int64_t m, const float* s_points, int64_t n_s,
+                                      const float* s_feats, int64_t c, int64_t ldf, const uint8_t* s_positive,
+                                      const int64_t* idx, int64_t h, int64_t ldi, const int32_t* width,
+                                      const float* kernel_points, float sigma, float* wf, int64_t ldw,
+                                      float* nn, const float* order_records, int32_t* mask, void* stream) {
+  return rdm::kpconv_gather_impl(q_points, m, s_points, n_s, s_feats, c, ldf, s_positive, idx, h, ldi, width, kernel_points, sigma,
+                                 wf, ldw, nn, order_records, 0, stream, 0, mask, nullptr);
+}
+
 extern "C" int rdm_kpconv_gather_ordered(const float* q_points, int64_t m, const float* s_points, int64_t n_s,
                                          const float* s_feats, int64_t c, int64_t ldf, const uint8_t* s_positive,
                                          const int64_t* idx, int64_t h, int64_t ldi, const int32_t* width,
diff --git a/rdmnet_amd/engine.py b/rdmnet_amd/engine.py
--- a/rdmnet_amd/engine.py
+++ b/rdmnet_amd/engine.py
@@ -135,6 +135,9 @@
 
     def set_overlap(self, mode=1):
         _lib.check(self.L.rdm_engine_set_overlap(self._h, int(mode)), 'rdm_engine_set_overlap')
+
+    def set_kpconv_zero_tiles(self, enable=True):
+        _lib.check(self.L.rdm_engine_set_kpconv_zero_tiles(self._h, int(enable)), 'rdm_engine_set_kpconv_zero_tiles')
 
     def reserve(self, arena_bytes):
         self.clear_pending()
```

New measurement: 624.2, median of 6. No clear change (+0.7%).
